# dantodor/Neural-Ficititious-Self-Play-in-Imperfect-Information-Games

Hardware: NVIDIA B200
Metric: leduc_transitions_per_sec (higher is better)
Workload: dtype f32

## Files before the change

include/nfsp_b200.h:

```cpp
#ifndef NFSP_B200_H
#define NFSP_B200_H
#include <stdint.h>

#ifdef __cplusplus
extern "C" {
#endif

#define NFSP_OK 0
#define NFSP_E_ARG (-1)
#define NFSP_E_CUDA (-2)
#define NFSP_E_STATE (-3)

#define NFSP_RULES_LEGACY 0
#define NFSP_RULES_NFSP 1

#define NFSP_OBS_DIM 30
#define NFSP_ACTIONS 3
#define NFSP_HIDDEN 64
#define NFSP_NET_PARAMS 2179
#define NFSP_EXPORT_FIELDS 24
#define NFSP_LEGACY_EXPORT_FIELDS 14
#define NFSP_STATS_FIELDS 16

typedef struct nfsp_env_s *nfsp_env_t;

int nfsp_version(void);
const char *nfsp_last_error(void);
int nfsp_device_info(int device, int *sm_count, int *cc_major, int *cc_minor, char *name, int name_len);

int nfsp_env_create(int rules, int64_t n_games, uint64_t seed, uint64_t game0, int device, nfsp_env_t *out);
int nfsp_env_destroy(nfsp_env_t h);
int64_t nfsp_env_num_games(nfsp_env_t h);
int nfsp_env_rules(nfsp_env_t h);
uint64_t nfsp_env_step_counter(nfsp_env_t h);
int nfsp_env_set_step_counter(nfsp_env_t h, uint64_t step);
void *nfsp_env_state_ptr(nfsp_env_t h);
int nfsp_env_kernel_error(nfsp_env_t h, uint32_t *out);
int nfsp_env_save_state(nfsp_env_t h, uint64_t *d_out, void *stream);
int nfsp_env_load_state(nfsp_env_t h, const uint64_t *d_in, void *stream);

int nfsp_env_reset(nfsp_env_t h, const int8_t *d_dealer, double eta, void *stream);
int nfsp_env_set_hands(nfsp_env_t h, const int8_t *d_dealer, const int8_t *d_cards, const int8_t *d_policy,
                       void *stream);
int nfsp_env_step(nfsp_env_t h, const int8_t *d_actions, const int8_t *d_players, int n_steps, int auto_reset,
                  double eta, uint32_t *d_trace, void *stream);
int nfsp_fsm_image(uint32_t *out, int capacity_words);
int nfsp_legacy_fsm_image(uint32_t *out, int capacity_words, int *n_rows);
int nfsp_rollout_image(uint32_t *out, int capacity_words);
int nfsp_env_do_action(nfsp_env_t h, const int8_t *d_actions, const int8_t *d_players, int8_t *d_fold, void *stream);
int nfsp_env_observe(nfsp_env_t h, const int8_t *d_players, int player, uint32_t *d_s, uint32_t *d_s2,
                     float *d_reward, uint8_t *d_term, uint8_t *d_last_a, void *stream);
int nfsp_env_export(nfsp_env_t h, int32_t *d_fields, void *stream);

int nfsp_legacy_reset(nfsp_env_t h, void *stream);
int nfsp_legacy_set_hands(nfsp_env_t h, const int8_t *d_cards, void *stream);
int nfsp_legacy_step(nfsp_env_t h, const int8_t *d_actions, const int8_t *d_players, int player, void *stream);
int nfsp_legacy_get_new_state(nfsp_env_t h, const int8_t *d_players, int player, int32_t *d_out, void *stream);
int nfsp_legacy_rollout(nfsp_env_t h, const int8_t *d_actions, int n_iters, uint32_t *d_rec, void *stream);
int nfsp_legacy_export(nfsp_env_t h, int32_t *d_fields, void *stream);

int nfsp_expand_obs(const uint32_t *d_masks, int64_t n, float *d_out, void *stream);

int nfsp_act_set_weights(nfsp_env_t h, const float *d_weights, void *stream);
int nfsp_act_set_weights_from_host(nfsp_env_t h, const float *h_weights, float *d_weights, void *stream);
int nfsp_act_forward(nfsp_env_t h, const uint32_t *d_obs, const int8_t *d_net, int64_t n, float *d_out,
                     void *stream);

int nfsp_act_forward_tc(nfsp_env_t h, const uint32_t *d_obs, const int8_t *d_net, int64_t n, float *d_out,
                        void *stream);

typedef struct {
    void *d_rl[2];
    void *d_sl[2];
    int64_t cap_rl, cap_sl;
    int32_t n_segments;
    uint32_t *d_counts;
    uint64_t *d_stats;
    uint32_t *d_trace;
    float *d_vec;
    const float *d_forced_vec;
    int32_t variant;
    int32_t reserve_sms;
    void *d_ring[2];
    uint64_t *d_ring_total[2];
    int64_t ring_cap;
    int32_t epsilon_per_player;
    double epsilon_p1;
} nfsp_rollout_io;
#define NFSP_ROLLOUT_DEFAULT_VARIANT 6

int nfsp_rollout(nfsp_env_t h, int n_steps, double eta, double epsilon, const nfsp_rollout_io *io, void *stream);
int nfsp_rollout_with_weights(nfsp_env_t h, const float *h_weights, float *d_weights, int n_steps, double eta, double epsilon,
                              const nfsp_rollout_io *io, void *stream);
int nfsp_rollout_tune(nfsp_env_t h, int patience_avg, int patience_br);
int nfsp_rollout_profile(nfsp_env_t h, uint64_t *out24);

#define NFSP_INSERT_SCRATCH_WORDS 4
int nfsp_ring_insert(void *d_ring, int64_t cap, uint64_t *d_total, const void *d_recs, uint32_t *d_counts,
                     int n_segments, int64_t seg_cap, uint64_t *d_scratch, void *stream);
#define NFSP_RESERVOIR_SLOT_BYTES 32
int nfsp_reservoir_insert(void *d_res, int64_t cap, uint64_t *d_total, const void *d_recs, uint32_t *d_counts,
                          int n_segments, int64_t seg_cap, uint64_t seed, int mode, uint64_t *d_scratch, void *stream);
#define NFSP_MAX_INSERT_REQS 4
typedef struct {
    void *d_mem;
    int64_t cap;
    uint64_t *d_total;
    uint64_t *d_scratch;
    const void *d_recs;
    uint32_t *d_counts;
    int32_t n_segments;
    int64_t seg_cap;
    uint64_t seed;
    int32_t mode;
    int32_t reservoir;
} nfsp_insert_req;
int nfsp_insert_multi(const nfsp_insert_req *reqs, int n, void *stream);
int nfsp_ring_insert_multi(const nfsp_insert_req *reqs, int n, void *stream);
int nfsp_reservoir_insert_multi(const nfsp_insert_req *reqs, int n, void *stream);
int nfsp_sample_indices(uint64_t seed, uint64_t call_idx, const uint64_t *d_total, int64_t cap, int is_ring,
                        int batch, int64_t *d_idx, uint32_t *d_n_out, void *stream);
#define NFSP_MAX_SAMPLE_REQS 8
typedef struct {
    const void *d_mem;
    const uint64_t *d_total;
    int64_t cap;
    uint64_t seed, call_idx;
    int32_t is_ring;
    float *d_out;
    void *d_rec_out;
} nfsp_sample_req;
int nfsp_sample_minibatches(const nfsp_sample_req *reqs, int n_reqs, int batch, int64_t *d_idx, uint32_t *d_n_out,
                            void *stream);
int nfsp_gather_rl(const void *d_ring, const int64_t *d_idx, int batch, float *d_s, float *d_a, float *d_r,
                   float *d_s2, float *d_t, void *stream);
int nfsp_gather_sl(const void *d_res, const int64_t *d_idx, int batch, float *d_s, float *d_a, void *stream);

#define NFSP_LEARNER_STATS 8
typedef struct {
    const float *d_weights;
    const float *d_target_weights;
    const void *d_rl[2];
    const int64_t *d_rl_idx[2];
    const void *d_sl[2];
    const int64_t *d_sl_idx[2];
    int32_t row0, rows;
    float gamma;
    int32_t net_mask;
    int32_t terminal_bootstraps;
    int32_t others_to_target;
    float *d_grad;
    float *d_stats;
} nfsp_learner_io;
int nfsp_learner_grads(const nfsp_learner_io *io, void *stream);
#define NFSP_MAX_FIT_STEPS 64
int nfsp_learner_fit(const nfsp_learner_io *io, int minibatch, int fit_batch, int epochs, const float lr[4],
                     float *d_weights_out, void *stream);
#define NFSP_MAX_PEERS 8
#define NFSP_PEER_BUF_FLOATS 279552
typedef struct {
    int32_t world, rank;
    void *d_buf[NFSP_MAX_PEERS];
    uint32_t epoch0;
    uint32_t *d_err;
    void *d_mc;
} nfsp_peers;
int nfsp_learner_fit_peers(const nfsp_learner_io *io, int minibatch, int fit_batch, int epochs, const float lr[4],
                           float *d_weights_out, const nfsp_peers *peers, void *stream);
int nfsp_peer_buffer_create(int device, void **d_buf, unsigned char *handle64);
int nfsp_peer_buffer_open(int device, const unsigned char *handle64, void **d_buf);
int nfsp_peer_buffer_close(int device, void *d_buf);
int nfsp_peer_buffer_destroy(int device, void *d_buf);
int nfsp_sgd_apply(float *d_weights, const float *d_grad, const float lr[4], float scale, void *stream);

#ifdef __cplusplus
}
#endif
#endif
```

neural-ficititious-self-play-in-imperfect-information-games_b200/_lib.py:

```python
from __future__ import annotations

import ctypes as C
import os

PKG_DIR = os.path.dirname(os.path.abspath(__file__))
LIB_PATH = os.path.join(PKG_DIR, "libnfsp_b200.so")

RULES_LEGACY, RULES_NFSP = 0, 1
OBS_DIM, ACTIONS, HIDDEN, NET_PARAMS = 30, 3, 64, 2179
EXPORT_FIELDS, LEGACY_EXPORT_FIELDS, STATS_FIELDS = 24, 14, 16

SYMBOLS = [
    "nfsp_version", "nfsp_last_error", "nfsp_device_info",
    "nfsp_env_create", "nfsp_env_destroy", "nfsp_env_num_games", "nfsp_env_rules", "nfsp_env_step_counter",
    "nfsp_env_set_step_counter", "nfsp_env_state_ptr", "nfsp_env_kernel_error", "nfsp_env_save_state", "nfsp_env_load_state",
    "nfsp_env_reset", "nfsp_env_set_hands", "nfsp_env_step", "nfsp_env_do_action", "nfsp_fsm_image", "nfsp_legacy_fsm_image", "nfsp_rollout_image", "nfsp_env_observe", "nfsp_env_export",
    "nfsp_legacy_reset", "nfsp_legacy_set_hands", "nfsp_legacy_step", "nfsp_legacy_get_new_state",
    "nfsp_legacy_rollout", "nfsp_legacy_export",
    "nfsp_expand_obs",
    "nfsp_act_set_weights", "nfsp_act_set_weights_from_host", "nfsp_act_forward", "nfsp_act_forward_tc", "nfsp_rollout", "nfsp_rollout_with_weights", "nfsp_rollout_tune", "nfsp_rollout_profile",
    "nfsp_ring_insert", "nfsp_reservoir_insert", "nfsp_insert_multi", "nfsp_ring_insert_multi", "nfsp_reservoir_insert_multi", "nfsp_sample_indices", "nfsp_sample_minibatches", "nfsp_gather_rl", "nfsp_gather_sl",
    "nfsp_learner_grads", "nfsp_learner_fit", "nfsp_learner_fit_peers", "nfsp_sgd_apply",
    "nfsp_peer_buffer_create", "nfsp_peer_buffer_open", "nfsp_peer_buffer_close", "nfsp_peer_buffer_destroy",
]


class RolloutIO(C.Structure):
    _fields_ = [("d_rl", C.c_void_p * 2), ("d_sl", C.c_void_p * 2), ("cap_rl", C.c_int64), ("cap_sl", C.c_int64),
                ("n_segments", C.c_int32), ("d_counts", C.c_void_p), ("d_stats", C.c_void_p), ("d_trace", C.c_void_p), ("d_vec", C.c_void_p),
                ("d_forced_vec", C.c_void_p), ("variant", C.c_int32), ("reserve_sms", C.c_int32),
                ("d_ring", C.c_void_p * 2), ("d_ring_total", C.c_void_p * 2), ("ring_cap", C.c_int64),
                ("epsilon_per_player", C.c_int32), ("epsilon_p1", C.c_double)]


class InsertReq(C.Structure):
    _fields_ = [("d_mem", C.c_void_p), ("cap", C.c_int64), ("d_total", C.c_void_p), ("d_scratch", C.c_void_p),
                ("d_recs", C.c_void_p), ("d_counts", C.c_void_p), ("n_segments", C.c_int32), ("seg_cap", C.c_int64),
                ("seed", C.c_uint64), ("mode", C.c_int32), ("reservoir", C.c_int32)]


INSERT_SCRATCH_WORDS, RESERVOIR_SLOT_BYTES = 4, 32


MAX_PEERS, PEER_BUF_FLOATS = 8, 279552


class Peers(C.Structure):
    _fields_ = [("world", C.c_int32), ("rank", C.c_int32), ("d_buf", C.c_void_p * MAX_PEERS), ("epoch0", C.c_uint32),
                ("d_err", C.c_void_p), ("d_mc", C.c_void_p)]


class SampleReq(C.Structure):
    _fields_ = [("d_mem", C.c_void_p), ("d_total", C.c_void_p), ("cap", C.c_int64), ("seed", C.c_uint64),
                ("call_idx", C.c_uint64), ("is_ring", C.c_int32), ("d_out", C.c_void_p), ("d_rec_out", C.c_void_p)]


class LearnerIO(C.Structure):
    _fields_ = [("d_weights", C.c_void_p), ("d_target_weights", C.c_void_p), ("d_rl", C.c_void_p * 2),
                ("d_rl_idx", C.c_void_p * 2), ("d_sl", C.c_void_p * 2), ("d_sl_idx", C.c_void_p * 2),
                ("row0", C.c_int32), ("rows", C.c_int32), ("gamma", C.c_float), ("net_mask", C.c_int32),
                ("terminal_bootstraps", C.c_int32), ("others_to_target", C.c_int32), ("d_grad", C.c_void_p), ("d_stats", C.c_void_p)]


class NfspError(RuntimeError):
    pass


_lib = None


def lib():
    global _lib
    if _lib is not None:
        return _lib
    if not os.path.exists(LIB_PATH):
        raise NfspError("libnfsp_b200.so is not built (%s): run `python -c 'import __graft_entry__ as g; g.build()'`; "
                        "there is no CPU fallback" % LIB_PATH)
    L = C.CDLL(LIB_PATH)
    vp, i8p = C.c_void_p, C.c_void_p
    L.nfsp_version.restype = C.c_int
    L.nfsp_last_error.restype = C.c_char_p
    L.nfsp_device_info.argtypes = [C.c_int, C.POINTER(C.c_int), C.POINTER(C.c_int), C.POINTER(C.c_int), C.c_char_p,
                                   C.c_int]
    L.nfsp_env_create.argtypes = [C.c_int, C.c_int64, C.c_uint64, C.c_uint64, C.c_int, C.POINTER(vp)]
    L.nfsp_env_destroy.argtypes = [vp]
    L.nfsp_env_num_games.argtypes = [vp]
    L.nfsp_env_num_games.restype = C.c_int64
    L.nfsp_env_rules.argtypes = [vp]
    L.nfsp_env_step_counter.argtypes = [vp]
    L.nfsp_env_step_counter.restype = C.c_uint64
    L.nfsp_env_set_step_counter.argtypes = [vp, C.c_uint64]
    L.nfsp_env_state_ptr.argtypes = [vp]
    L.nfsp_env_state_ptr.restype = vp
    L.nfsp_env_kernel_error.argtypes = [vp, C.POINTER(C.c_uint32)]
    L.nfsp_rollout_tune.argtypes = [vp, C.c_int, C.c_int]
    L.nfsp_rollout_profile.argtypes = [vp, C.POINTER(C.c_uint64)]
    L.nfsp_env_save_state.argtypes = [vp, vp, vp]
    L.nfsp_env_load_state.argtypes = [vp, vp, vp]
    L.nfsp_env_reset.argtypes = [vp, i8p, C.c_double, vp]
    L.nfsp_env_set_hands.argtypes = [vp, i8p, i8p, i8p, vp]
    L.nfsp_env_step.argtypes = [vp, i8p, i8p, C.c_int, C.c_int, C.c_double, vp, vp]
    L.nfsp_env_do_action.argtypes = [vp, i8p, i8p, i8p, vp]
    L.nfsp_fsm_image.argtypes = [vp, C.c_int]
    L.nfsp_legacy_fsm_image.argtypes = [vp, C.c_int, vp]
    L.nfsp_rollout_image.argtypes = [vp, C.c_int]
    L.nfsp_env_observe.argtypes = [vp, i8p, C.c_int, vp, vp, vp, vp, vp, vp]
    L.nfsp_env_export.argtypes = [vp, vp, vp]
    L.nfsp_legacy_reset.argtypes = [vp, vp]
    L.nfsp_legacy_set_hands.argtypes = [vp, i8p, vp]
    L.nfsp_legacy_step.argtypes = [vp, i8p, i8p, C.c_int, vp]
    L.nfsp_legacy_get_new_state.argtypes = [vp, i8p, C.c_int, vp, vp]
    L.nfsp_legacy_rollout.argtypes = [vp, i8p, C.c_int, vp, vp]
    L.nfsp_legacy_export.argtypes = [vp, vp, vp]
    L.nfsp_expand_obs.argtypes = [vp, C.c_int64, vp, vp]
    L.nfsp_act_set_weights.argtypes = [vp, vp, vp]
    L.nfsp_act_set_weights_from_host.argtypes = [vp, vp, vp, vp]
    L.nfsp_act_forward.argtypes = [vp, vp, i8p, C.c_int64, vp, vp]
    L.nfsp_act_forward_tc.argtypes = [vp, vp, i8p, C.c_int64, vp, vp]
    L.nfsp_rollout.argtypes = [vp, C.c_int, C.c_double, C.c_double, C.POINTER(RolloutIO), vp]
    L.nfsp_rollout_with_weights.argtypes = [vp, vp, vp, C.c_int, C.c_double, C.c_double, C.POINTER(RolloutIO), vp]
    L.nfsp_ring_insert.argtypes = [vp, C.c_int64, vp, vp, vp, C.c_int, C.c_int64, vp, vp]
    L.nfsp_reservoir_insert.argtypes = [vp, C.c_int64, vp, vp, vp, C.c_int, C.c_int64, C.c_uint64, C.c_int, vp, vp]
    L.nfsp_insert_multi.argtypes = [C.POINTER(InsertReq), C.c_int, vp]
    L.nfsp_ring_insert_multi.argtypes = [C.POINTER(InsertReq), C.c_int, vp]
    L.nfsp_reservoir_insert_multi.argtypes = [C.POINTER(InsertReq), C.c_int, vp]
    L.nfsp_sample_indices.argtypes = [C.c_uint64, C.c_uint64, vp, C.c_int64, C.c_int, C.c_int, vp, vp, vp]
    L.nfsp_sample_minibatches.argtypes = [C.POINTER(SampleReq), C.c_int, C.c_int, vp, vp, vp]
    L.nfsp_gather_rl.argtypes = [vp, vp, C.c_int, vp, vp, vp, vp, vp, vp]
    L.nfsp_gather_sl.argtypes = [vp, vp, C.c_int, vp, vp, vp]
    L.nfsp_learner_grads.argtypes = [C.POINTER(LearnerIO), vp]
    L.nfsp_learner_fit.argtypes = [C.POINTER(LearnerIO), C.c_int, C.c_int, C.c_int, C.POINTER(C.c_float), vp, vp]
    L.nfsp_learner_fit_peers.argtypes = [C.POINTER(LearnerIO), C.c_int, C.c_int, C.c_int, C.POINTER(C.c_float), vp,
                                         C.POINTER(Peers), vp]
    L.nfsp_sgd_apply.argtypes = [vp, vp, C.POINTER(C.c_float * 4), C.c_float, vp]
    L.nfsp_peer_buffer_create.argtypes = [C.c_int, C.POINTER(vp), C.c_char_p]
    L.nfsp_peer_buffer_open.argtypes = [C.c_int, C.c_char_p, C.POINTER(vp)]
    L.nfsp_peer_buffer_close.argtypes = [C.c_int, vp]
    L.nfsp_peer_buffer_destroy.argtypes = [C.c_int, vp]
    _lib = L
    return L


def check(rc: int):
    if rc != 0:
        raise NfspError("libnfsp_b200 error %d: %s" % (rc, lib().nfsp_last_error().decode("utf-8", "replace")))
```

neural-ficititious-self-play-in-imperfect-information-games_b200/csrc/act_kernels.cu:

```cuda
#include "mlp_math.cuh"
#include "ptx_helpers.cuh"
#include "rollout_fast.cuh"
#include "rollout_tables.cuh"

namespace nfsp {

constexpr int kActThreads = 128;
constexpr int kRollThreads = 1024;
constexpr int kFwdRowQuads = 24;
constexpr int kW1Floats = 128 * kFwdRowQuads * 4;
constexpr int kW2Floats = 4 * 3 * kFwdRowQuads * 4;
constexpr int kPackFloats = kW1Floats + kW2Floats + kB2Floats;

__device__ __forceinline__ float pack_weights_value(const float *__restrict__ w, int e) {
    {
        float v = 0.f;
        if (e < kW1Floats) {
            const int c = e & 3, pos = (e >> 2) % kFwdRowQuads, row = (e >> 2) / kFwdRowQuads;
            const int net = row >> 5, i = row & 31, j = (pos & 15) * 4 + c;
            const float *wn = w + net * NFSP_NET_PARAMS;
            if (i < 30) v = wn[i * 64 + j];
            else if (i == 30) v = wn[1920 + j];
        } else if (e < kW1Floats + kW2Floats) {
            const int f = e - kW1Floats, x = f & 3, pos = (f >> 2) % kFwdRowQuads, c = ((f >> 2) / kFwdRowQuads) % 3;
            const int net = (f >> 2) / (3 * kFwdRowQuads);
            v = w[net * NFSP_NET_PARAMS + 1984 + ((pos & 15) * 4 + x) * 3 + c];
        } else {
            const int f = e - kW1Floats - kW2Floats, c = f & 3, net = f >> 2;
            if (c < 3) v = w[net * NFSP_NET_PARAMS + 2176 + c];
        }
        return v;
    }
}

static_assert((kPackFloats + kTabImageFloats + 4 * NFSP_NET_PARAMS) % 4 == 0, "the state table behind the images must be 16-byte aligned (bulk copy)");
__global__ void pack_images_kernel(const float *__restrict__ w, float *__restrict__ pack) {
    constexpr int kImages = kPackFloats + kTabImageFloats;
    for (int e = blockIdx.x * blockDim.x + threadIdx.x; e < kImages + 4 * NFSP_NET_PARAMS; e += gridDim.x * blockDim.x)
        pack[e] = e < kPackFloats ? pack_weights_value(w, e) : (e < kImages ? pack_tables_value(w, e - kPackFloats) : w[e - kImages]);
}

__device__ __forceinline__ void mlp_forward(const float *__restrict__ sw, uint32_t obs, int net, uint32_t rot, float out[3]) {
    const float4 *w1 = reinterpret_cast<const float4 *>(sw) + rot;
    float4 h[16];
#pragma unroll
    for (int q = 0; q < 16; ++q) h[q] = make_float4(0.f, 0.f, 0.f, 0.f);
    uint32_t bits = (obs & 0x3FFFFFFFu) | (1u << 30);
    while (bits) {
        const int i = __ffs(bits) - 1;
        bits &= bits - 1u;
        const float4 *r = w1 + (net * 32 + i) * kFwdRowQuads;
#pragma unroll
        for (int q = 0; q < 16; ++q) {
            const float4 v = r[q];
            h[q].x += v.x; h[q].y += v.y; h[q].z += v.z; h[q].w += v.w;
        }
    }
    const float4 *w2 = reinterpret_cast<const float4 *>(sw + kW1Floats) + net * (3 * kFwdRowQuads) + rot;
    Layer2Acc acc;
#pragma unroll
    for (int q = 0; q < 16; ++q)
        acc.quad(h[q].x, h[q].y, h[q].z, h[q].w, w2[q], w2[kFwdRowQuads + q], w2[2 * kFwdRowQuads + q]);
    acc.head(reinterpret_cast<const float4 *>(sw + kW1Floats + kW2Floats)[net], net & 1, out[0], out[1], out[2]);
}

__device__ __forceinline__ void load_pack(float *sw, const float *__restrict__ pack) {
    const float4 *src = reinterpret_cast<const float4 *>(pack);
    float4 *dst = reinterpret_cast<float4 *>(sw);
    for (int e = threadIdx.x; e < kPackFloats / 4; e += blockDim.x) dst[e] = src[e];
    __syncthreads();
}

__global__ void __launch_bounds__(kActThreads)
act_forward_kernel(const float *__restrict__ pack, const uint32_t *__restrict__ obs, const int8_t *__restrict__ net,
                   int64_t n, float *__restrict__ out) {
    extern __shared__ __align__(16) float sw[];
    load_pack(sw, pack);
    for (int64_t i = blockIdx.x * (int64_t)blockDim.x + threadIdx.x; i < n; i += (int64_t)gridDim.x * blockDim.x) {
        float v[3];
        mlp_forward(sw, obs[i], (int)(net[i] & 3), (uint32_t)i & 7u, v);
        out[3 * i] = v[0]; out[3 * i + 1] = v[1]; out[3 * i + 2] = v[2];
    }
}

template <bool kDebug, bool kDirect>
__global__ void __launch_bounds__(kRollThreads, 1)
rollout_kernel(const RolloutArgs A) {
    extern __shared__ __align__(128) float sw[];
    __shared__ unsigned long long s_stats[NFSP_STATS_FIELDS];
    __shared__ __align__(8) uint64_t s_bar;
    __shared__ FastLuts s_lut;
    __shared__ uint32_t s_next;
    if (threadIdx.x < NFSP_STATS_FIELDS) s_stats[threadIdx.x] = 0ull;
    s_lut.fill();
    const uint32_t bar = smem_u32(&s_bar);
    if (threadIdx.x == 0) {
        s_next = 0u;
        mbar_init(bar, 1);
        fence_mbar_init();
    }
    __syncthreads();
    if (threadIdx.x == 0) {
        mbar_expect_tx(bar, kTabImageBytes);
        constexpr uint32_t kChunk = 32768;
        for (uint32_t off = 0; off < (uint32_t)kTabImageBytes; off += kChunk) {
            const uint32_t len = (uint32_t)kTabImageBytes - off < kChunk ? (uint32_t)kTabImageBytes - off : kChunk;
            bulk_g2s(smem_u32(sw) + off, reinterpret_cast<const uint8_t *>(A.pack) + off, len, bar);
        }
    }
    bool image_ready = false;

    FastCounters c;
    const int64_t plane = (int64_t)A.n_steps * A.n;
    const uint32_t lane = threadIdx.x & 31u;
    const int64_t n_blocks = (A.n + 31) >> 5;
    for (;;) {
        uint32_t blk = 0;
        if (lane == 0) blk = blockIdx.x + gridDim.x * atomicAdd(&s_next, 1u);
        blk = __shfl_sync(0xFFFFFFFFu, blk, 0);
        if ((int64_t)blk >= n_blocks) break;
        const int64_t base = (int64_t)blk << 5;
        const int64_t i = base + lane;
        const bool live = i < A.n;
        const uint64_t game = A.game0 + (uint64_t)i;
        const uint32_t rot = (uint32_t)game & 7u;
        WarpStage W;
        W.init(A, (uint32_t)(base >> 5) & (A.n_seg - 1u), kDirect);
        NfspFast g;
        g.unpack(live ? A.state[i] : 0ull);
        for (int t = 0; t < A.n_steps; ++t) {
            FastDecision d;
            fast_begin(g, s_lut, A, game, A.step0 + (uint64_t)t, live, d, c);
            const uint32_t sg = g.sigma(), dl = g.dealer(), ca = (g.PA >> 11) & 3u;
            const uint32_t xrow = sg >= 9u ? 3u + ((((ca * 3u + g.pub()) * 2u + dl) << 2) | g.fin0()) : ca;
            const uint32_t yrow = 75u + dl * 18u + sg;
            float v0, v1, v2;
            if (!image_ready) {
                mbar_wait(bar, 0);
                image_ready = true;
            }
            mlp_forward_tables(sw, xrow, yrow, g.p() * 2u + (uint32_t)d.pol, rot, v0, v1, v2);
            if (d.random) { v0 = d.r0; v1 = d.r1; v2 = d.r2; }
            fast_finish<kDebug, kDirect>(g, s_lut, A, W, d, v0, v1, v2, live, (int64_t)t * A.n + i, plane, c);
            if ((t & 15) == 15) c.spill();
        }
        c.spill();
        if (live) A.state[i] = g.pack();
        c.wide.trans += live ? A.n_steps : 0;
    }
    if (!image_ready) mbar_wait(bar, 0);
    c.spill();
    if (A.stats) c.wide.commit(s_stats, A.stats);
}

}

using namespace nfsp;

extern "C" int nfsp_act_set_weights(nfsp_env_t h, const float *d_weights, void *stream) {
    NFSP_CHECK_ARG(h != nullptr && d_weights != nullptr, "null argument");
    NFSP_CHECK_ARG(h->rules == NFSP_RULES_NFSP, "acting nets need NFSP rules");
    DeviceGuard guard(h->device);
    if (!guard.ok) return set_error(NFSP_E_CUDA, "cannot select device %d", h->device);
    if (!h->d_wpack) {
        NFSP_CUDA(cudaMalloc(&h->d_wpack, sizeof(float) * (kPackFloats + kTabImageFloats + 4 * NFSP_NET_PARAMS + nfsp_states_floats())));
        h->d_wcopy = h->d_wpack + kPackFloats + kTabImageFloats;
        h->d_states = h->d_wpack + kPackFloats + kTabImageFloats + 4 * NFSP_NET_PARAMS;
        NFSP_CUDA(cudaMalloc(&h->d_work, sizeof(uint32_t)));
        NFSP_CUDA(cudaFuncSetAttribute(act_forward_kernel, cudaFuncAttributeMaxDynamicSharedMemorySize, (int)(kPackFloats * sizeof(float))));
        NFSP_CUDA(cudaFuncSetAttribute(rollout_kernel<true, false>, cudaFuncAttributeMaxDynamicSharedMemorySize, kTabImageBytes));
        NFSP_CUDA(cudaFuncSetAttribute(rollout_kernel<false, false>, cudaFuncAttributeMaxDynamicSharedMemorySize, kTabImageBytes));
        NFSP_CUDA(cudaFuncSetAttribute(rollout_kernel<true, true>, cudaFuncAttributeMaxDynamicSharedMemorySize, kTabImageBytes));
        NFSP_CUDA(cudaFuncSetAttribute(rollout_kernel<false, true>, cudaFuncAttributeMaxDynamicSharedMemorySize, kTabImageBytes));
        int rc = nfsp_rollout_sorted_configure();
        if (rc != NFSP_OK) return rc;
        rc = nfsp_rollout_pairs_configure();
        if (rc != NFSP_OK) return rc;
        rc = nfsp_rollout_states_configure();
        if (rc != NFSP_OK) return rc;
        rc = nfsp_states_upload_image(h->d_states);
        if (rc != NFSP_OK) return rc;
    }
    pack_images_kernel<<<(kPackFloats + kTabImageFloats + 4 * NFSP_NET_PARAMS + 255) / 256, 256, 0, (cudaStream_t)stream>>>(d_weights, h->d_wpack);
    NFSP_LAUNCH_CHECK();
    h->tc_dirty = h->tq_dirty = h->st_dirty = true;
    h->has_weights = true;
    return nfsp_states_ensure(h, h->d_wpack + kPackFloats, h->d_states, (cudaStream_t)stream);
}

int nfsp_ensure_tc_images(nfsp_env_t h, bool tq, cudaStream_t st) {
    if (h->tc_dirty) {
        const int rc = nfsp_pack_tc_image(h, h->d_wcopy, st);
        if (rc != NFSP_OK) return rc;
        h->tc_dirty = false;
    }
    if (tq && h->tq_dirty) {
        const int rc = nfsp_tq_set_weights(h, h->d_wcopy, st);
        if (rc != NFSP_OK) return rc;
        h->tq_dirty = false;
    }
    return NFSP_OK;
}

extern "C" int nfsp_act_set_weights_from_host(nfsp_env_t h, const float *h_weights, float *d_weights, void *stream) {
    NFSP_CHECK_ARG(h != nullptr && h_weights != nullptr && d_weights != nullptr, "null argument");
    DeviceGuard guard(h->device);
    if (!guard.ok) return set_error(NFSP_E_CUDA, "cannot select device %d", h->device);
    NFSP_CUDA(cudaMemcpyAsync(d_weights, h_weights, sizeof(float) * 4 * NFSP_NET_PARAMS, cudaMemcpyHostToDevice,
                              (cudaStream_t)stream));
    return nfsp_act_set_weights(h, d_weights, stream);
}

extern "C" int nfsp_act_forward(nfsp_env_t h, const uint32_t *d_obs, const int8_t *d_net, int64_t n, float *d_out,
                                void *stream) {
    NFSP_CHECK_ARG(h != nullptr && d_obs && d_net && d_out && n >= 0, "bad arguments");
    if (!h->has_weights) return set_error(NFSP_E_STATE, "nfsp_act_set_weights has not been called");
    if (n == 0) return NFSP_OK;
    DeviceGuard guard(h->device);
    if (!guard.ok) return set_error(NFSP_E_CUDA, "cannot select device %d", h->device);
    const int grid = grid_for(n, kActThreads, h->sm_count, 4);
    act_forward_kernel<<<grid, kActThreads, kPackFloats * sizeof(float), (cudaStream_t)stream>>>(h->d_wpack, d_obs, d_net, n, d_out);
    NFSP_LAUNCH_CHECK();
    return NFSP_OK;
}

int nfsp_rollout_direct_args(const nfsp_rollout_io *io, RolloutArgs &A, bool *direct) {
    for (int q = 0; q < 2; ++q) { A.ring[q] = nullptr; A.ring_total[q] = nullptr; }
    A.ring_cap = 0u;
    A.ring_magic = 0ull;
    *direct = io->d_ring[0] != nullptr || io->d_ring[1] != nullptr;
    if (!*direct) return NFSP_OK;
    NFSP_CHECK_ARG(io->d_ring[0] && io->d_ring[1] && io->d_ring_total[0] && io->d_ring_total[1],
                   "the direct ring append needs both rings and their totals");
    NFSP_CHECK_ARG(io->ring_cap > 1 && io->ring_cap < ((int64_t)1 << 32), "ring capacity out of range");
    NFSP_CHECK_ARG(2 * A.n * (int64_t)A.n_steps <= io->ring_cap,
                   "direct ring append needs 2 * n * n_steps <= ring capacity (a launch must not lap the ring)");
    for (int q = 0; q < 2; ++q) {
        A.ring[q] = (uint4 *)io->d_ring[q];
        A.ring_total[q] = (unsigned long long *)io->d_ring_total[q];
    }
    A.ring_cap = (uint32_t)io->ring_cap;
    A.ring_magic = ~0ull / (uint64_t)io->ring_cap;
    return NFSP_OK;
}

extern "C" int nfsp_rollout(nfsp_env_t h, int n_steps, double eta, double epsilon, const nfsp_rollout_io *io,
                            void *stream) {
    NFSP_CHECK_ARG(h != nullptr && io != nullptr, "null argument");
    NFSP_CHECK_ARG(h->rules == NFSP_RULES_NFSP, "rollout needs NFSP rules");
    NFSP_CHECK_ARG(n_steps >= 1 && n_steps <= 4096, "n_steps must be in [1,4096]");
    NFSP_CHECK_ARG(io->d_rl[0] && io->d_rl[1] && io->d_sl[0] && io->d_sl[1] && io->d_counts, "missing staging arrays");
    NFSP_CHECK_ARG(io->cap_rl > 0 && io->cap_sl > 0 && io->cap_rl < ((int64_t)1 << 32) && io->cap_sl < ((int64_t)1 << 32),
                   "staging capacity out of range");
    NFSP_CHECK_ARG(io->n_segments >= 1 && io->n_segments <= 65536 && (io->n_segments & (io->n_segments - 1)) == 0,
                   "n_segments must be a power of two in [1,65536]");
    if (!h->has_weights) return set_error(NFSP_E_STATE, "nfsp_act_set_weights has not been called");
    DeviceGuard guard(h->device);
    if (!guard.ok) return set_error(NFSP_E_CUDA, "cannot select device %d", h->device);
    RolloutArgs A;
    A.keys = philox_keys(h->seed);
    A.state = h->d_state; A.n = h->n; A.seed = h->seed; A.game0 = h->game0; A.step0 = h->step; A.n_steps = n_steps;
    A.eta_u32 = frac_u32(eta); A.eps_u32 = frac_u32(epsilon);
    A.eps1_u32 = io->epsilon_per_player ? frac_u32(io->epsilon_p1) : A.eps_u32;
    A.pack = h->d_wpack + kPackFloats;
    for (int q = 0; q < 2; ++q) { A.rl[q] = (uint4 *)io->d_rl[q]; A.sl[q] = (uint4 *)io->d_sl[q]; }
    A.cap_rl = io->cap_rl; A.cap_sl = io->cap_sl; A.n_seg = (uint32_t)io->n_segments; A.counts = io->d_counts;
    A.work = h->d_work;
    A.stats = (unsigned long long *)io->d_stats; A.trace = io->d_trace; A.vec = io->d_vec; A.forced = io->d_forced_vec;
    const bool debug = io->d_trace || io->d_vec || io->d_forced_vec;
    NFSP_CHECK_ARG(io->variant >= 0 && io->variant <= 6,
                   "variant must be 0 (default), 1 (CUDA cores), 2 (tcgen05, one tile per group), 3 (tcgen05, warp-specialised), "
                   "4 (CUDA cores, net-sorted groups), 5 (CUDA cores, two games per lane) or 6 (table of the nets' outputs per decision state)");
    const int variant = io->variant == 0 ? NFSP_ROLLOUT_DEFAULT_VARIANT : io->variant;
    NFSP_CHECK_ARG(io->reserve_sms >= 0 && io->reserve_sms < h->sm_count, "reserve_sms must be in [0, %d)", h->sm_count);
    bool direct = false;
    {
        const int rc = nfsp_rollout_direct_args(io, A, &direct);
        if (rc != NFSP_OK) return rc;
    }
    NFSP_CHECK_ARG(!direct || variant == 1 || variant >= 4, "the direct ring append (d_ring) exists in variants 1, 4, 5 and 6 only");
    if (variant == 6) {
        int rc = nfsp_states_ensure(h, h->d_wpack + kPackFloats, h->d_states, (cudaStream_t)stream);
        if (rc != NFSP_OK) return rc;
        A.pack = h->d_states;
        rc = nfsp_rollout_states_launch(h, A, io, debug, (cudaStream_t)stream);
        if (rc != NFSP_OK) return rc;
        h->step += (uint64_t)n_steps;
        return NFSP_OK;
    }
    if (variant == 5) {
        const int rc = nfsp_rollout_pairs_launch(h, A, io, debug, (cudaStream_t)stream);
        if (rc != NFSP_OK) return rc;
        h->step += (uint64_t)n_steps;
        return NFSP_OK;
    }
    if (variant == 4) {
        const int rc = nfsp_rollout_sorted_launch(h, A, io, debug, (cudaStream_t)stream);
        if (rc != NFSP_OK) return rc;
        h->step += (uint64_t)n_steps;
        return NFSP_OK;
    }
    if (variant == 2 || variant == 3) {
        const int rc = nfsp_ensure_tc_images(h, variant == 3, (cudaStream_t)stream);
        if (rc != NFSP_OK) return rc;
    }
    if (variant == 3) {
        const int rc = nfsp_rollout_tq_launch(h, A, debug, io->reserve_sms, (cudaStream_t)stream);
        if (rc != NFSP_OK) return rc;
        h->step += (uint64_t)n_steps;
        return NFSP_OK;
    }
    if (variant == 2) {
        const int rc = nfsp_rollout_tc_launch(h, A, debug, (cudaStream_t)stream);
        if (rc != NFSP_OK) return rc;
        h->step += (uint64_t)n_steps;
        return NFSP_OK;
    }
    const int grid = grid_for(h->n, 32, h->sm_count - io->reserve_sms, 1);
    if (debug && direct) rollout_kernel<true, true><<<grid, kRollThreads, kTabImageBytes, (cudaStream_t)stream>>>(A);
    else if (debug) rollout_kernel<true, false><<<grid, kRollThreads, kTabImageBytes, (cudaStream_t)stream>>>(A);
    else if (direct) rollout_kernel<false, true><<<grid, kRollThreads, kTabImageBytes, (cudaStream_t)stream>>>(A);
    else rollout_kernel<false, false><<<grid, kRollThreads, kTabImageBytes, (cudaStream_t)stream>>>(A);
    NFSP_LAUNCH_CHECK();
    h->step += (uint64_t)n_steps;
    return NFSP_OK;
}

extern "C" int nfsp_rollout_with_weights(nfsp_env_t h, const float *h_weights, float *d_weights, int n_steps, double eta,
                                         double epsilon, const nfsp_rollout_io *io, void *stream) {
    const int rc = h_weights ? nfsp_act_set_weights_from_host(h, h_weights, d_weights, stream) : nfsp_act_set_weights(h, d_weights, stream);
    if (rc != NFSP_OK) return rc;
    return nfsp_rollout(h, n_steps, eta, epsilon, io, stream);
}
```

neural-ficititious-self-play-in-imperfect-information-games_b200/csrc/buffer_kernels.cu:

```cuda
#include <cstdlib>

#include "common.cuh"
#include "philox.cuh"

namespace nfsp {

constexpr int kBufThreads = 256;

__device__ __forceinline__ uint64_t mulhi64(uint64_t a, uint64_t b) { return __umul64hi(a, b); }

struct Batch {
    const uint4 *recs;
    uint32_t *counts;
    uint32_t n_seg;
    uint64_t seg_cap;
};

struct Mem {
    uint4 *data;
    uint64_t cap;
    uint64_t *total;
    uint64_t *scratch;
    Batch B;
    uint64_t seed;
    int mode;
    int reservoir;
};
struct MemSet {
    Mem m[NFSP_MAX_INSERT_REQS];
    int n;
    uint32_t gx;
    uint64_t chunk;
    int small;
};
constexpr int kScratchHead = 2;
constexpr uint64_t kResChunk = 1ull << 21;

__device__ __forceinline__ void grid_sync(uint64_t *ctrl) {
    __syncthreads();
    if (threadIdx.x == 0) {
        unsigned long long *cnt = reinterpret_cast<unsigned long long *>(ctrl);
        volatile unsigned long long *gen = reinterpret_cast<volatile unsigned long long *>(ctrl + 1);
        const unsigned long long g = *gen;
        __threadfence();
        if (atomicAdd(cnt, 1ull) == (unsigned long long)gridDim.x - 1ull) {
            *cnt = 0ull;
            __threadfence();
            atomicAdd(const_cast<unsigned long long *>(gen), 1ull);
        } else {
            while (*gen == g) __nanosleep(32);
        }
        __threadfence();
    }
    __syncthreads();
}

__device__ __forceinline__ void scan_counts(const Mem &M) {
    __shared__ unsigned long long s_warp[kBufThreads / 32];
    __shared__ unsigned long long s_run;
    if (threadIdx.x == 0) s_run = 0ull;
    __syncthreads();
    uint64_t *pre = M.scratch + kScratchHead;
    const uint32_t lane = threadIdx.x & 31u, warp = threadIdx.x >> 5;
    for (uint32_t k0 = 0; k0 < M.B.n_seg; k0 += kBufThreads) {
        const uint32_t k = k0 + threadIdx.x;
        unsigned long long c = 0ull;
        if (k < M.B.n_seg) {
            c = M.B.counts[k];
            if (c > M.B.seg_cap) c = M.B.seg_cap;
        }
        unsigned long long incl = c;
#pragma unroll
        for (int o = 1; o < 32; o <<= 1) {
            const unsigned long long up = __shfl_up_sync(0xFFFFFFFFu, incl, o);
            if (lane >= (uint32_t)o) incl += up;
        }
        if (lane == 31) s_warp[warp] = incl;
        __syncthreads();
        unsigned long long before = s_run;
        for (uint32_t w = 0; w < warp; ++w) before += s_warp[w];
        if (k < M.B.n_seg) pre[k] = before + incl - c;
        __syncthreads();
        if (threadIdx.x == kBufThreads - 1) s_run = before + incl;
        __syncthreads();
    }
    if (threadIdx.x == 0) pre[M.B.n_seg] = s_run;
}

constexpr int kRingUnroll = 4;
__device__ __forceinline__ void ring_item(const Mem &M, uint64_t total, uint32_t seg, uint32_t x, uint32_t gx, uint64_t before,
                                          uint64_t cnt, uint64_t m) {
    const Batch &B = M.B;
    const uint64_t cap = M.cap;
    const uint64_t first = m > cap ? m - cap : 0;
    const uint4 *src = B.recs + (uint64_t)seg * B.seg_cap;
    uint4 *ring = M.data;
    const uint64_t head = total % cap;
    const uint64_t stride = (uint64_t)gx * blockDim.x;
    for (uint64_t i0 = x * (uint64_t)blockDim.x + threadIdx.x; i0 < cnt; i0 += stride * kRingUnroll) {
        uint4 v[kRingUnroll];
#pragma unroll
        for (int u = 0; u < kRingUnroll; ++u) {
            const uint64_t i = i0 + (uint64_t)u * stride;
            if (i < cnt) v[u] = __ldcs(src + i);
        }
#pragma unroll
        for (int u = 0; u < kRingUnroll; ++u) {
            const uint64_t i = i0 + (uint64_t)u * stride, idx = before + i;
            if (i < cnt && idx >= first) {
                uint64_t slot = head + idx;
                if (slot >= cap) slot -= cap;
                if (slot >= cap) slot %= cap;
                ring[slot] = v[u];
            }
        }
    }
}

__device__ __forceinline__ int64_t reservoir_slot(uint64_t seed, uint64_t ticket, uint64_t cap, int mode) {
    if (ticket < cap) return (int64_t)ticket;
    const uint64_t u = buffer_u64(seed, ticket, 0, STREAM_RESERVOIR);
    if (mode == 1) {
        const uint64_t j = 1u + mulhi64(u, cap);
        return j < cap ? (int64_t)j : -1;
    }
    const uint64_t j = mulhi64(u, ticket + 1u);
    return j < cap ? (int64_t)j : -1;
}

constexpr int kResUnroll = 4;

template <bool kWrite>
__device__ __forceinline__ void reservoir_item(const Mem &M, uint64_t total, uint32_t seg, uint32_t x, uint32_t gx, uint64_t lo,
                                               uint64_t hi, uint64_t before, uint64_t cnt) {
    const Batch &B = M.B;
    if (before >= hi || before + cnt <= lo) return;
    const uint64_t i_lo = lo > before ? lo - before : 0, i_hi = hi - before < cnt ? hi - before : cnt;
    const uint64_t cap = M.cap, seed = M.seed;
    const int mode = M.mode;
    uint4 *res = M.data;
    const uint4 *src = B.recs + (uint64_t)seg * B.seg_cap;
    const uint64_t stride = (uint64_t)gx * blockDim.x;
    for (uint64_t i0 = i_lo + x * (uint64_t)blockDim.x + threadIdx.x; i0 < i_hi; i0 += stride * kResUnroll) {
        int64_t slot[kResUnroll];
#pragma unroll
        for (int u = 0; u < kResUnroll; ++u) {
            const uint64_t i = i0 + (uint64_t)u * stride;
            slot[u] = i < i_hi ? reservoir_slot(seed, total + before + i, cap, mode) : -1;
        }
        if (!kWrite) {
#pragma unroll
            for (int u = 0; u < kResUnroll; ++u)
                if (slot[u] >= 0)
                    atomicMax(reinterpret_cast<unsigned long long *>(res + 2 * slot[u] + 1),
                              (unsigned long long)(total + before + i0 + (uint64_t)u * stride + 1u));
        } else {
            unsigned long long owner[kResUnroll];
#pragma unroll
            for (int u = 0; u < kResUnroll; ++u)
                owner[u] = slot[u] >= 0 ? __ldcg(reinterpret_cast<const unsigned long long *>(res + 2 * slot[u] + 1)) : 0ull;
#pragma unroll
            for (int u = 0; u < kResUnroll; ++u) {
                const uint64_t i = i0 + (uint64_t)u * stride;
                if (slot[u] >= 0 && owner[u] == (unsigned long long)(total + before + i + 1u)) res[2 * slot[u]] = __ldcs(src + i);
            }
        }
    }
}

template <class F>
__device__ __forceinline__ void for_items(const MemSet &S, int k, const uint64_t *pre, bool in_smem, F f) {
    const uint64_t items = (uint64_t)S.m[k].B.n_seg * S.gx;
    for (uint64_t w = blockIdx.x; w < items; w += gridDim.x) {
        const uint32_t seg = (uint32_t)(w / S.gx), x = (uint32_t)(w % S.gx);
        const uint64_t before = in_smem ? pre[seg] : __ldcg(pre + seg), next = in_smem ? pre[seg + 1] : __ldcg(pre + seg + 1);
        f(seg, x, before, next - before);
    }
}

constexpr int kSmallSegs = 32;

__global__ void __launch_bounds__(kBufThreads, 4) insert_kernel(const MemSet S) {
    __shared__ uint64_t s_pre[NFSP_MAX_INSERT_REQS][kSmallSegs + 1];
    uint64_t *ctrl = S.m[0].scratch;
    uint64_t total[NFSP_MAX_INSERT_REQS], m_all[NFSP_MAX_INSERT_REQS];
    const uint64_t *pre[NFSP_MAX_INSERT_REQS];
    const bool small = S.small != 0;
#pragma unroll
    for (int k = 0; k < NFSP_MAX_INSERT_REQS; ++k) total[k] = k < S.n ? *S.m[k].total : 0ull;
    if (small) {
        const uint32_t lane = threadIdx.x & 31u, warp = threadIdx.x >> 5;
        if (warp < (uint32_t)S.n) {
            const Mem &M = S.m[warp];
            unsigned long long c = lane < M.B.n_seg ? (unsigned long long)__ldcg(M.B.counts + lane) : 0ull;
            if (c > M.B.seg_cap) c = M.B.seg_cap;
            unsigned long long incl = c;
#pragma unroll
            for (int o = 1; o < 32; o <<= 1) {
                const unsigned long long up = __shfl_up_sync(0xFFFFFFFFu, incl, o);
                if (lane >= (uint32_t)o) incl += up;
            }
            s_pre[warp][lane + 1] = incl;
            if (lane == 0) s_pre[warp][0] = 0ull;
        }
        __syncthreads();
#pragma unroll
        for (int k = 0; k < NFSP_MAX_INSERT_REQS; ++k) {
            pre[k] = s_pre[k];
            m_all[k] = k < S.n ? s_pre[k][S.m[k].B.n_seg] : 0ull;
        }
    } else {
        for (int k = blockIdx.x; k < S.n; k += gridDim.x) scan_counts(S.m[k]);
        grid_sync(ctrl);
#pragma unroll
        for (int k = 0; k < NFSP_MAX_INSERT_REQS; ++k) {
            pre[k] = k < S.n ? S.m[k].scratch + kScratchHead : nullptr;
            m_all[k] = k < S.n ? __ldcg(pre[k] + S.m[k].B.n_seg) : 0ull;
        }
    }
    uint64_t res_max = 0;
#pragma unroll
    for (int k = 0; k < NFSP_MAX_INSERT_REQS; ++k)
        if (k < S.n && S.m[k].reservoir) res_max = m_all[k] > res_max ? m_all[k] : res_max;
#pragma unroll
    for (int k = 0; k < NFSP_MAX_INSERT_REQS; ++k)
        if (k < S.n && !S.m[k].reservoir)
            for_items(S, k, pre[k], small, [&](uint32_t seg, uint32_t x, uint64_t before, uint64_t cnt) {
                ring_item(S.m[k], total[k], seg, x, S.gx, before, cnt, m_all[k]);
            });
    for (uint64_t lo = 0; lo < res_max; lo += S.chunk) {
#pragma unroll
        for (int k = 0; k < NFSP_MAX_INSERT_REQS; ++k)
            if (k < S.n && S.m[k].reservoir)
                for_items(S, k, pre[k], small, [&](uint32_t seg, uint32_t x, uint64_t before, uint64_t cnt) {
                    reservoir_item<false>(S.m[k], total[k], seg, x, S.gx, lo, lo + S.chunk, before, cnt);
                });
        grid_sync(ctrl);
#pragma unroll
        for (int k = 0; k < NFSP_MAX_INSERT_REQS; ++k)
            if (k < S.n && S.m[k].reservoir)
                for_items(S, k, pre[k], small, [&](uint32_t seg, uint32_t x, uint64_t before, uint64_t cnt) {
                    reservoir_item<true>(S.m[k], total[k], seg, x, S.gx, lo, lo + S.chunk, before, cnt);
                });
    }
    if (small && res_max == 0) grid_sync(ctrl);
#pragma unroll
    for (int k = 0; k < NFSP_MAX_INSERT_REQS; ++k)
        if (k < S.n && (uint32_t)k % gridDim.x == blockIdx.x) {
            const Mem &M = S.m[k];
            for (uint32_t s = threadIdx.x; s < M.B.n_seg; s += blockDim.x) M.B.counts[s] = 0u;
            if (threadIdx.x == 0) *M.total = total[k] + m_all[k];
        }
}

constexpr int kMaxBatch = 1024;

template <class SlotT>
__device__ __forceinline__ int floyd_sample(uint64_t seed, uint64_t call_idx, uint64_t total, uint64_t cap, int is_ring,
                                            int batch, uint64_t *draw, uint64_t *pick, SlotT *slot_out) {
    __shared__ int s_collision;
    const uint64_t count = total < cap ? total : cap;
    const int b = (uint64_t)batch < count ? batch : (int)count;
    const uint64_t lo = count - (uint64_t)b;
    if (threadIdx.x == 0) s_collision = 0;
    for (int m = threadIdx.x; m < b; m += blockDim.x)
        draw[m] = mulhi64(buffer_u64(seed, (uint64_t)m, call_idx, STREAM_SAMPLE), lo + (uint64_t)m + 1u);
    __syncthreads();
    __shared__ unsigned char s_dup[kMaxBatch];
    for (int m = threadIdx.x; m < b; m += blockDim.x) {
        const uint64_t t = draw[m];
        bool dup = false;
        for (int k = 0; k < m; ++k) dup |= (draw[k] == t);
        if (dup) s_collision = 1;
        s_dup[m] = dup;
    }
    __syncthreads();
    while (s_collision) {
        __syncthreads();
        if (threadIdx.x == 0) s_collision = 0;
        __syncthreads();
        for (int m = threadIdx.x; m < b; m += blockDim.x) {
            const uint64_t t = draw[m];
            if (!s_dup[m] && t >= lo && t - lo < (uint64_t)m && s_dup[t - lo]) {
                s_dup[m] = 1;
                s_collision = 1;
            }
        }
        __syncthreads();
    }
    for (int m = threadIdx.x; m < b; m += blockDim.x) pick[m] = s_dup[m] ? lo + (uint64_t)m : draw[m];
    __syncthreads();
    const uint64_t head = (is_ring && total >= cap) ? total % cap : 0;
    for (int m = threadIdx.x; m < batch; m += blockDim.x) {
        int64_t slot = -1;
        if (m < b) slot = is_ring ? (int64_t)((head + pick[m]) % cap) : (int64_t)pick[m];
        slot_out[m] = (SlotT)slot;
    }
    return b;
}

__global__ void __launch_bounds__(kBufThreads)
sample_kernel(uint64_t seed, uint64_t call_idx, const uint64_t *__restrict__ total_p, uint64_t cap, int is_ring,
              int batch, int64_t *__restrict__ idx_out, uint32_t *__restrict__ n_out) {
    __shared__ uint64_t draw[kMaxBatch];
    __shared__ uint64_t pick[kMaxBatch];
    const int b = floyd_sample(seed, call_idx, *total_p, cap, is_ring, batch, draw, pick, idx_out);
    if (threadIdx.x == 0 && n_out) *n_out = (uint32_t)b;
}

__device__ __forceinline__ void expand_rl(const uint4 rec, int row, int col, float *__restrict__ s, float *__restrict__ a,
                                          float *__restrict__ r, float *__restrict__ s2, float *__restrict__ t) {
    if (col < 30) s[row * 30 + col] = (float)((rec.x >> col) & 1u);
    else if (col < 60) s2[row * 30 + (col - 30)] = (float)((rec.y >> (col - 30)) & 1u);
    else if (col < 63) a[row * 3 + (col - 60)] = ((rec.w & 0xFFu) == (uint32_t)(col - 60)) ? 1.f : 0.f;
    else if (col == 63) r[row] = __uint_as_float(rec.z);
    else t[row] = (float)((rec.w >> 8) & 0xFFu);
}
__device__ __forceinline__ void expand_sl(const uint4 rec, int row, int col, float *__restrict__ s, float *__restrict__ a) {
    if (col < 30) s[row * 30 + col] = (float)((rec.x >> col) & 1u);
    else a[row * 3 + (col - 30)] = __uint_as_float(col == 30 ? rec.y : (col == 31 ? rec.z : rec.w));
}

struct SampleReqs {
    const uint4 *mem[NFSP_MAX_SAMPLE_REQS];
    const uint64_t *total[NFSP_MAX_SAMPLE_REQS];
    uint64_t cap[NFSP_MAX_SAMPLE_REQS], seed[NFSP_MAX_SAMPLE_REQS], call_idx[NFSP_MAX_SAMPLE_REQS];
    float *out[NFSP_MAX_SAMPLE_REQS];
    uint4 *rec_out[NFSP_MAX_SAMPLE_REQS];
    int is_ring[NFSP_MAX_SAMPLE_REQS];
};
__global__ void __launch_bounds__(kBufThreads)
sample_gather_kernel(const SampleReqs R, int batch, int64_t *__restrict__ idx_out, uint32_t *__restrict__ n_out) {
    __shared__ uint64_t draw[kMaxBatch];
    __shared__ uint64_t pick[kMaxBatch];
    __shared__ int64_t slot[kMaxBatch];
    __shared__ uint4 s_rec[kMaxBatch];
    const int m = blockIdx.x;
    const int b = floyd_sample(R.seed[m], R.call_idx[m], *R.total[m], R.cap[m], R.is_ring[m], batch, draw, pick, slot);
    __syncthreads();
    const int per = (batch + (int)gridDim.y - 1) / (int)gridDim.y;
    const int row0 = (int)blockIdx.y * per, row1 = min(batch, row0 + per);
    if (threadIdx.x == 0 && blockIdx.y == 0 && n_out) n_out[m] = (uint32_t)b;
    const uint4 *mem = R.mem[m];
    float *o = R.out[m];
    uint4 *ro = R.rec_out[m];
    const int stride = R.is_ring[m] ? 1 : 2;
    for (int k = row0 + threadIdx.x; k < row1; k += blockDim.x) {
        if (idx_out) idx_out[(int64_t)m * batch + k] = slot[k];
        if (o || ro) {
            const uint4 rec = slot[k] >= 0 ? mem[slot[k] * stride] : make_uint4(0, 0, 0, 0);
            if (o) s_rec[k] = rec;
            if (ro) ro[k * stride] = rec;
        }
    }
    if (!o) return;
    __syncthreads();
    const int rows = max(row1 - row0, 0);
    if (R.is_ring[m]) {
        float *s = o, *a = s + 30 * batch, *r = a + 3 * batch, *s2 = r + batch, *t = s2 + 30 * batch;
        for (int e = threadIdx.x; e < rows * 65; e += blockDim.x) {
            const int row = row0 + e / 65, col = e % 65;
            expand_rl(s_rec[row], row, col, s, a, r, s2, t);
        }
    } else {
        float *s = o, *a = s + 30 * batch;
        for (int e = threadIdx.x; e < rows * 33; e += blockDim.x) {
            const int row = row0 + e / 33, col = e % 33;
            expand_sl(s_rec[row], row, col, s, a);
        }
    }
}

__global__ void __launch_bounds__(kBufThreads)
gather_rl_kernel(const uint4 *__restrict__ ring, const int64_t *__restrict__ idx, int batch, float *__restrict__ s,
                 float *__restrict__ a, float *__restrict__ r, float *__restrict__ s2, float *__restrict__ t) {
    const int total = batch * 65;
    for (int e = blockIdx.x * blockDim.x + threadIdx.x; e < total; e += gridDim.x * blockDim.x) {
        const int row = e / 65, col = e - row * 65;
        const int64_t slot = idx[row];
        expand_rl(slot >= 0 ? ring[slot] : make_uint4(0, 0, 0, 0), row, col, s, a, r, s2, t);
    }
}

__global__ void __launch_bounds__(kBufThreads)
gather_sl_kernel(const uint4 *__restrict__ res, const int64_t *__restrict__ idx, int batch, float *__restrict__ s,
                 float *__restrict__ a) {
    const int total = batch * 33;
    for (int e = blockIdx.x * blockDim.x + threadIdx.x; e < total; e += gridDim.x * blockDim.x) {
        const int row = e / 33, col = e - row * 33;
        const int64_t slot = idx[row];
        expand_sl(slot >= 0 ? res[2 * slot] : make_uint4(0, 0, 0, 0), row, col, s, a);
    }
}

}

using namespace nfsp;

static int make_memset(const nfsp_insert_req *reqs, int n, int want_kind, MemSet &S, int64_t *seg_cap_max) {
    NFSP_CHECK_ARG(reqs && n >= 1 && n <= NFSP_MAX_INSERT_REQS, "1..%d memories per call", NFSP_MAX_INSERT_REQS);
    *seg_cap_max = 0;
    int64_t rows = 0;
    for (int k = 0; k < NFSP_MAX_INSERT_REQS; ++k) S.m[k] = Mem{};
    for (int k = 0; k < n; ++k) {
        const nfsp_insert_req &r = reqs[k];
        NFSP_CHECK_ARG(r.d_mem && r.d_total && r.cap > 0, "bad memory %d", k);
        NFSP_CHECK_ARG(r.d_recs && r.d_counts && r.d_scratch, "null staged batch or scratch %d", k);
        NFSP_CHECK_ARG(r.n_segments >= 1 && r.n_segments <= 65535 && r.seg_cap >= 0, "bad segment geometry %d", k);
        NFSP_CHECK_ARG(r.reservoir == 0 || r.reservoir == 1, "reservoir must be 0 (ring) or 1 (reservoir)");
        NFSP_CHECK_ARG(want_kind < 0 || r.reservoir == want_kind, "memory %d is of the other kind", k);
        if (r.reservoir) NFSP_CHECK_ARG(r.mode == 0 || r.mode == 1, "mode must be 0 (Algorithm R) or 1 (reference law)");
        S.m[k].data = (uint4 *)r.d_mem;
        S.m[k].cap = (uint64_t)r.cap;
        S.m[k].total = r.d_total;
        S.m[k].scratch = r.d_scratch;
        S.m[k].B = Batch{(const uint4 *)r.d_recs, r.d_counts, (uint32_t)r.n_segments, (uint64_t)r.seg_cap};
        S.m[k].seed = r.seed;
        S.m[k].mode = r.mode;
        S.m[k].reservoir = r.reservoir;
        if (r.seg_cap > *seg_cap_max) *seg_cap_max = r.seg_cap;
        rows += r.n_segments;
    }
    S.n = n;
    int64_t g = (*seg_cap_max + kBufThreads - 1) / kBufThreads;
    const int64_t lim = rows >= 148 * 8 ? 1 : (148 * 8 + rows - 1) / rows;
    if (g > lim) g = lim;
    if (g < 1) g = 1;
    S.gx = (uint32_t)g;
    S.small = 1;
    for (int k = 0; k < n; ++k)
        if (reqs[k].n_segments > 32) S.small = 0;
    S.chunk = kResChunk;
#ifdef NFSP_TUNING_HOOKS
    if (const char *e = getenv("NFSP_RES_CHUNK")) {
        const long long v = atoll(e);
        if (v >= 1024) S.chunk = (uint64_t)v;
    }
#endif
    return NFSP_OK;
}

static int launch_insert(MemSet &S, cudaStream_t st) {
    int dev = 0, sms = 0, per_sm = 0;
    NFSP_CUDA(cudaGetDevice(&dev));
    NFSP_CUDA(cudaDeviceGetAttribute(&sms, cudaDevAttrMultiProcessorCount, dev));
    NFSP_CUDA(cudaOccupancyMaxActiveBlocksPerMultiprocessor(&per_sm, insert_kernel, kBufThreads, 0));
    if (per_sm < 1) return set_error(NFSP_E_CUDA, "insert_kernel does not fit an SM");
    if (per_sm > 8) per_sm = 8;
    int64_t items = 0;
    for (int k = 0; k < S.n; ++k) items += (int64_t)S.m[k].B.n_seg * S.gx;
    int64_t grid = (int64_t)sms * per_sm;
    if (items < grid) grid = items;
    if (grid < S.n) grid = S.n;
    void *args[] = {(void *)&S};
    NFSP_CUDA(cudaLaunchCooperativeKernel((const void *)insert_kernel, dim3((unsigned)grid), dim3(kBufThreads), args, 0, st));
    return NFSP_OK;
}

extern "C" int nfsp_insert_multi(const nfsp_insert_req *reqs, int n, void *stream) {
    MemSet S;
    int64_t seg_cap;
    const int rc = make_memset(reqs, n, -1, S, &seg_cap);
    if (rc != NFSP_OK) return rc;
    if (seg_cap == 0) return NFSP_OK;
    return launch_insert(S, (cudaStream_t)stream);
}

extern "C" int nfsp_ring_insert_multi(const nfsp_insert_req *reqs, int n, void *stream) {
    MemSet S;
    int64_t seg_cap;
    const int rc = make_memset(reqs, n, 0, S, &seg_cap);
    if (rc != NFSP_OK) return rc;
    if (seg_cap == 0) return NFSP_OK;
    return launch_insert(S, (cudaStream_t)stream);
}

extern "C" int nfsp_reservoir_insert_multi(const nfsp_insert_req *reqs, int n, void *stream) {
    MemSet S;
    int64_t seg_cap;
    const int rc = make_memset(reqs, n, 1, S, &seg_cap);
    if (rc != NFSP_OK) return rc;
    if (seg_cap == 0) return NFSP_OK;
    return launch_insert(S, (cudaStream_t)stream);
}

extern "C" int nfsp_ring_insert(void *d_ring, int64_t cap, uint64_t *d_total, const void *d_recs, uint32_t *d_counts,
                                int n_segments, int64_t seg_cap, uint64_t *d_scratch, void *stream) {
    nfsp_insert_req r{};
    r.d_mem = d_ring; r.cap = cap; r.d_total = d_total; r.d_recs = d_recs; r.d_counts = d_counts;
    r.n_segments = n_segments; r.seg_cap = seg_cap; r.d_scratch = d_scratch;
    return nfsp_ring_insert_multi(&r, 1, stream);
}

extern "C" int nfsp_reservoir_insert(void *d_res, int64_t cap, uint64_t *d_total, const void *d_recs, uint32_t *d_counts,
                                     int n_segments, int64_t seg_cap, uint64_t seed, int mode, uint64_t *d_scratch,
                                     void *stream) {
    nfsp_insert_req r{};
    r.d_mem = d_res; r.cap = cap; r.d_total = d_total; r.d_recs = d_recs; r.d_counts = d_counts;
    r.n_segments = n_segments; r.seg_cap = seg_cap; r.seed = seed; r.mode = mode; r.d_scratch = d_scratch; r.reservoir = 1;
    return nfsp_reservoir_insert_multi(&r, 1, stream);
}

extern "C" int nfsp_sample_indices(uint64_t seed, uint64_t call_idx, const uint64_t *d_total, int64_t cap,
                                   int is_ring, int batch, int64_t *d_idx, uint32_t *d_n_out, void *stream) {
    NFSP_CHECK_ARG(d_total && d_idx && cap > 0, "bad arguments");
    NFSP_CHECK_ARG(batch >= 1 && batch <= kMaxBatch, "batch must be in [1,%d]", kMaxBatch);
    sample_kernel<<<1, kBufThreads, 0, (cudaStream_t)stream>>>(seed, call_idx, d_total, (uint64_t)cap, is_ring, batch,
                                                               d_idx, d_n_out);
    NFSP_LAUNCH_CHECK();
    return NFSP_OK;
}

extern "C" int nfsp_sample_minibatches(const nfsp_sample_req *reqs, int n_reqs, int batch, int64_t *d_idx, uint32_t *d_n_out,
                                       void *stream) {
    NFSP_CHECK_ARG(reqs && n_reqs >= 1 && n_reqs <= NFSP_MAX_SAMPLE_REQS, "1..%d requests", NFSP_MAX_SAMPLE_REQS);
    NFSP_CHECK_ARG(batch >= 1 && batch <= kMaxBatch, "batch must be in [1,%d]", kMaxBatch);
    SampleReqs R;
    for (int m = 0; m < n_reqs; ++m) {
        NFSP_CHECK_ARG(reqs[m].d_mem && reqs[m].d_total && reqs[m].cap > 0, "bad request %d", m);
        NFSP_CHECK_ARG(reqs[m].d_out || reqs[m].d_rec_out || d_idx, "request %d has neither an output block nor an index array", m);
        R.mem[m] = (const uint4 *)reqs[m].d_mem;
        R.total[m] = reqs[m].d_total;
        R.cap[m] = (uint64_t)reqs[m].cap;
        R.seed[m] = reqs[m].seed;
        R.call_idx[m] = reqs[m].call_idx;
        R.out[m] = reqs[m].d_out;
        R.rec_out[m] = (uint4 *)reqs[m].d_rec_out;
        R.is_ring[m] = reqs[m].is_ring;
    }
    sample_gather_kernel<<<dim3((unsigned)n_reqs, 8u, 1u), kBufThreads, 0, (cudaStream_t)stream>>>(R, batch, d_idx, d_n_out);
    NFSP_LAUNCH_CHECK();
    return NFSP_OK;
}

extern "C" int nfsp_gather_rl(const void *d_ring, const int64_t *d_idx, int batch, float *d_s, float *d_a, float *d_r,
                              float *d_s2, float *d_t, void *stream) {
    NFSP_CHECK_ARG(d_ring && d_idx && d_s && d_a && d_r && d_s2 && d_t && batch >= 1, "bad arguments");
    gather_rl_kernel<<<(batch * 65 + kBufThreads - 1) / kBufThreads, kBufThreads, 0, (cudaStream_t)stream>>>(
        (const uint4 *)d_ring, d_idx, batch, d_s, d_a, d_r, d_s2, d_t);
    NFSP_LAUNCH_CHECK();
    return NFSP_OK;
}

extern "C" int nfsp_gather_sl(const void *d_res, const int64_t *d_idx, int batch, float *d_s, float *d_a,
                              void *stream) {
    NFSP_CHECK_ARG(d_res && d_idx && d_s && d_a && batch >= 1, "bad arguments");
    gather_sl_kernel<<<(batch * 33 + kBufThreads - 1) / kBufThreads, kBufThreads, 0, (cudaStream_t)stream>>>(
        (const uint4 *)d_res, d_idx, batch, d_s, d_a);
    NFSP_LAUNCH_CHECK();
    return NFSP_OK;
}
```

neural-ficititious-self-play-in-imperfect-information-games_b200/csrc/common.cuh:

```cuda
#pragma once
#include <cuda_runtime.h>

#include <cstdarg>
#include <cstdint>
#include <cstdio>

#include "../../include/nfsp_b200.h"

struct nfsp_env_s {
    int rules;
    int device;
    int sm_count;
    int64_t n;
    uint64_t seed, game0, step;
    uint64_t *d_state;
    uint32_t *d_fsm;
    float *d_wpack;
    uint32_t *d_work;
    void *d_wtc_wide;
    bool has_weights;
    bool tc_dirty = false, tq_dirty = false;
    bool st_dirty = false;
    float *d_states = nullptr;
    const float *d_wcopy = nullptr;
    int w2_slot = -1;
    void *d_w2img = nullptr;
    uint32_t *d_err = nullptr;
    uint32_t tq_patience[2] = {1500u, 700u};
};

int nfsp_fsm_upload(nfsp_env_t h);

int nfsp_pack_tc_image(nfsp_env_t h, const float *d_weights, cudaStream_t st);
int nfsp_ensure_tc_images(nfsp_env_t h, bool tq, cudaStream_t st);
int nfsp_tq_set_weights(nfsp_env_t h, const float *d_weights, cudaStream_t st);
void nfsp_tq_release(nfsp_env_t h);

namespace nfsp {

int set_error(int code, const char *fmt, ...);

#define NFSP_CHECK_ARG(cond, ...)                                    \
    do {                                                             \
        if (!(cond)) return nfsp::set_error(NFSP_E_ARG, __VA_ARGS__); \
    } while (0)

#define NFSP_CUDA(call)                                                                                   \
    do {                                                                                                  \
        cudaError_t e__ = (call);                                                                         \
        if (e__ != cudaSuccess)                                                                           \
            return nfsp::set_error(NFSP_E_CUDA, "%s failed: %s (%s:%d)", #call, cudaGetErrorString(e__), \
                                   __FILE__, __LINE__);                                                   \
    } while (0)

#define NFSP_LAUNCH_CHECK() NFSP_CUDA(cudaGetLastError())

inline uint32_t frac_u32(double x) {
    if (!(x > 0.0)) return 0u;
    const double v = x * 4294967296.0;
    return v >= 4294967295.0 ? 0xFFFFFFFFu : (uint32_t)v;
}

inline int grid_for(int64_t n, int threads, int sm_count, int ctas_per_sm) {
    const int64_t need = (n + threads - 1) / threads;
    const int64_t full = (int64_t)sm_count * ctas_per_sm;
    int64_t g = need < full ? need : full;
    if (g < 1) g = 1;
    return (int)g;
}

struct DeviceGuard {
    int prev = -1;
    bool ok = true;
    explicit DeviceGuard(int dev) {
        if (cudaGetDevice(&prev) != cudaSuccess) ok = false;
        if (ok && prev != dev && cudaSetDevice(dev) != cudaSuccess) ok = false;
    }
    ~DeviceGuard() {
        if (prev >= 0) cudaSetDevice(prev);
    }
};

}
```

neural-ficititious-self-play-in-imperfect-information-games_b200/csrc/ptx_helpers.cuh:

```cuda
#pragma once
#include <cstdint>

namespace nfsp {

__device__ __forceinline__ uint32_t smem_u32(const void *p) { return (uint32_t)__cvta_generic_to_shared(p); }

__device__ __forceinline__ void mbar_init(uint32_t bar, uint32_t count) {
    asm volatile("mbarrier.init.shared::cta.b64 [%0], %1;" ::"r"(bar), "r"(count));
}
__device__ __forceinline__ void mbar_expect_tx(uint32_t bar, uint32_t bytes) {
    asm volatile("mbarrier.arrive.expect_tx.shared::cta.b64 _, [%0], %1;" ::"r"(bar), "r"(bytes) : "memory");
}
__device__ __forceinline__ void mbar_wait(uint32_t bar, uint32_t parity) {
    asm volatile(
        "{\n\t"
        ".reg .pred p;\n\t"
        "WAIT_%=:\n\t"
        "mbarrier.try_wait.parity.shared::cta.b64 p, [%0], %1;\n\t"
        "@p bra DONE_%=;\n\t"
        "bra WAIT_%=;\n\t"
        "DONE_%=:\n\t"
        "}" ::"r"(bar), "r"(parity) : "memory");
}
__device__ __forceinline__ void mbar_wait_backoff(uint32_t bar, uint32_t parity) {
    uint32_t done = 0;
    while (true) {
        asm volatile(
            "{\n\t"
            ".reg .pred p;\n\t"
            "mbarrier.try_wait.parity.shared::cta.b64 p, [%1], %2;\n\t"
            "selp.u32 %0, 1, 0, p;\n\t"
            "}" : "=r"(done) : "r"(bar), "r"(parity) : "memory");
        if (done) break;
        __nanosleep(64);
    }
}
__device__ __forceinline__ void bulk_g2s(uint32_t dst, const void *src, uint32_t bytes, uint32_t bar) {
    asm volatile("cp.async.bulk.shared::cluster.global.mbarrier::complete_tx::bytes [%0], [%1], %2, [%3];" ::"r"(dst),
                 "l"(src), "r"(bytes), "r"(bar)
                 : "memory");
}
__device__ __forceinline__ void fence_mbar_init() { asm volatile("fence.mbarrier_init.release.cluster;" ::: "memory"); }

}
```

neural-ficititious-self-play-in-imperfect-information-games_b200/csrc/rollout_common.cuh:

```cuda
#pragma once
#include "common.cuh"
#include "nfsp_rules.cuh"
#include "philox.cuh"

namespace nfsp { struct RolloutArgs; }
int nfsp_rollout_tc_launch(nfsp_env_t h, const nfsp::RolloutArgs &A, bool debug, cudaStream_t st);
int nfsp_rollout_tq_launch(nfsp_env_t h, const nfsp::RolloutArgs &A, bool debug, int reserve_sms, cudaStream_t st);

int nfsp_rollout_sorted_launch(nfsp_env_t h, const nfsp::RolloutArgs &A, const nfsp_rollout_io *io, bool debug, cudaStream_t st);
int nfsp_rollout_direct_args(const nfsp_rollout_io *io, nfsp::RolloutArgs &A, bool *direct);
int nfsp_rollout_sorted_configure();
int nfsp_rollout_pairs_launch(nfsp_env_t h, const nfsp::RolloutArgs &A, const nfsp_rollout_io *io, bool debug, cudaStream_t st);
int nfsp_rollout_pairs_configure();

int nfsp_rollout_states_launch(nfsp_env_t h, const nfsp::RolloutArgs &A, const nfsp_rollout_io *io, bool debug, cudaStream_t st);
int nfsp_states_ensure(nfsp_env_t h, const float *d_tab, float *d_states, cudaStream_t st);
int nfsp_states_floats();
int nfsp_states_upload_image(float *d_states);
int nfsp_rollout_states_configure();

namespace nfsp {

struct RolloutArgs {
    uint64_t *state;
    int64_t n;
    uint64_t seed, game0, step0;
    PhiloxKeys keys;
    int n_steps;
    uint32_t eta_u32, eps_u32, eps1_u32;
    const void *pack;
    uint4 *rl[2];
    uint4 *sl[2];
    int64_t cap_rl, cap_sl;
    uint32_t n_seg;
    uint32_t *counts;
    uint32_t *work;
    unsigned long long *stats;
    uint32_t *trace;
    float *vec;
    const float *forced;
    uint4 *ring[2];
    unsigned long long *ring_total[2];
    uint32_t ring_cap;
    uint64_t ring_magic;
};

__device__ __forceinline__ uint32_t ring_slot(unsigned long long ticket, uint32_t cap, uint64_t magic) {
    const unsigned long long q = __umul64hi(ticket, magic);
    unsigned long long r = ticket - q * cap;
    if (r >= cap) r -= cap;
    return (uint32_t)r;
}

struct Counters {
    unsigned long long act0 = 0ull, act1 = 0ull;
    int rew0 = 0, rew1 = 0, hands = 0, trans = 0, drop = 0;

    __device__ __forceinline__ void commit(unsigned long long *s_stats, unsigned long long *g_stats) {
        long long v[11] = {(long long)(act0 & 0x1FFFFFull), (long long)((act0 >> 21) & 0x1FFFFFull), (long long)(act0 >> 42),
                           (long long)(act1 & 0x1FFFFFull), (long long)((act1 >> 21) & 0x1FFFFFull), (long long)(act1 >> 42),
                           rew0, rew1, hands, trans, drop};
#pragma unroll
        for (int k = 0; k < 11; ++k) {
#pragma unroll
            for (int o = 16; o > 0; o >>= 1) v[k] += __shfl_xor_sync(0xFFFFFFFFu, v[k], o);
        }
        if ((threadIdx.x & 31) == 0) {
#pragma unroll
            for (int k = 0; k < 11; ++k)
                if (v[k]) atomicAdd(&s_stats[k < 6 ? k : k + 2], (unsigned long long)v[k]);
        }
        act0 = act1 = 0ull;
        __syncthreads();
        if (threadIdx.x == 6) s_stats[6] = s_stats[0] + s_stats[1] + s_stats[2];
        if (threadIdx.x == 7) s_stats[7] = s_stats[3] + s_stats[4] + s_stats[5];
        __syncthreads();
        if (threadIdx.x < 13 && s_stats[threadIdx.x]) atomicAdd(g_stats + threadIdx.x, s_stats[threadIdx.x]);
    }
};

}
```

neural-ficititious-self-play-in-imperfect-information-games_b200/csrc/rollout_states.cu:

```cuda
#include "nfsp_fsm.cuh"
#include "rollout_fast.cuh"
#include "rollout_tables.cuh"
#include "ptx_helpers.cuh"

namespace nfsp {

constexpr int kNetStates = 72 * 18;
constexpr int kStateQuads = 4 * kNetStates;
constexpr int kStateBytes = kStateQuads * 16;
static_assert(kStateBytes % 16 == 0, "bulk copies move multiples of 16 bytes");
static_assert(kNetStates == fsm::kNetSlots, "the rollout image addresses this table");

__device__ __forceinline__ uint32_t score_word(float v0, float v1, float v2) {
    const uint32_t an = score_action(v0, v1, v2);
    return (an & 3u) * (uint32_t)fsm::kEntryBytes | (an >> 2) << 15;
}
constexpr uint32_t kWordEntry = 0x60u, kWordNz = 1u << 15;

__device__ __forceinline__ void state_rows(int s, uint32_t &xrow, uint32_t &yrow) {
    const uint32_t sg = (uint32_t)s % 18u, x = (uint32_t)s / 18u, dl = (x >> 2) & 1u;
    xrow = sg >= 9u ? 3u + x : x / 24u;
    yrow = 75u + dl * 18u + sg;
}

__global__ void states_pack_kernel(const float *__restrict__ tab, float4 *__restrict__ states) {
    const int t = blockIdx.x * blockDim.x + threadIdx.x, e = t >> 2, j = t & 3;
    const bool valid = e < kStateQuads;
    uint32_t xrow, yrow;
    state_rows(valid ? e % kNetStates : 0, xrow, yrow);
    const uint32_t net = valid ? (uint32_t)(e / kNetStates) : 0u;
    const float4 *T = reinterpret_cast<const float4 *>(tab);
    const float4 *xr = T + (net * kNetRows + xrow) * kRowQuads, *yr = T + (net * kNetRows + yrow) * kRowQuads;
    const float4 *wr = T + kTabRows * kRowQuads + net * (3 * kRowQuads);
    Layer2Acc acc;
#pragma unroll
    for (int k = 0; k < 4; ++k) {
        const int q = j + 4 * k;
        acc.quad_sum(xr[q], yr[q], wr[q], wr[kRowQuads + q], wr[2 * kRowQuads + q]);
    }
    float s0 = hsum2(acc.z0), s1 = hsum2(acc.z1), s2 = hsum2(acc.z2);
#pragma unroll
    for (int o = 1; o < 4; o <<= 1) {
        s0 += __shfl_xor_sync(0xFFFFFFFFu, s0, o);
        s1 += __shfl_xor_sync(0xFFFFFFFFu, s1, o);
        s2 += __shfl_xor_sync(0xFFFFFFFFu, s2, o);
    }
    if (valid && j == 0) {
        float o0, o1, o2;
        Layer2Acc::head_of_sums(s0, s1, s2, reinterpret_cast<const float4 *>(tab + kTabFloats + kTabW2Floats)[net], net & 1u, o0, o1, o2);
        states[e] = make_float4(o0, o1, o2, __uint_as_float(score_word(o0, o1, o2)));
    }
}

constexpr int kStatesThreads = 1024, kStatesThreadsSmall = 512;

constexpr int kBufRL = 100, kBufSL = 32;
constexpr int kWarpBufQuads = 2 * kBufRL + 2 * kBufSL;
constexpr int kImageQuads = fsm::kRImageBytes / 16;
constexpr int states_smem_bytes(int threads) { return kStateBytes + fsm::kRImageBytes + (threads / 32) * kWarpBufQuads * 16; }
static_assert(fsm::kRImageBytes % 16 == 0, "the warps' buffers follow the image 16-byte aligned");
static_assert(kBufRL >= 64 && kBufSL >= 32, "a buffer must take the records of one step");

constexpr uint32_t kOffRL1 = kBufRL, kOffSL0 = 2 * kBufRL, kOffSL1 = 2 * kBufRL + kBufSL;

struct WarpBuf {
    uint4 *b;
    uint32_t cnt = 0u;
};

__device__ __forceinline__ uint32_t warp_scan_bytes_p(uint32_t v) {
#pragma unroll
    for (int o = 1; o < 32; o <<= 1)
        asm volatile("{ .reg .pred p; .reg .u32 r; shfl.sync.up.b32 r|p, %0, %1, 0, 0xffffffff; @p add.u32 %0, %0, r; }" : "+r"(v) : "r"(o));
    return v;
}

template <bool kRing, int kCap>
__device__ __forceinline__ void buf_copy(const uint4 *src, uint32_t n, uint4 *dst, uint32_t base, uint32_t cap, int &drop) {
    const uint32_t lane = threadIdx.x & 31u;
#pragma unroll
    for (int it = 0; it < (kCap + 31) / 32; ++it) {
        const uint32_t k = lane + 32u * it;
        if (k < n) {
            uint32_t off = base + k;
            if (kRing) {
                off = off < cap ? off : off - cap;
                dst[off] = src[k];
            } else if (off < cap) {
                dst[off] = src[k];
            } else {
                ++drop;
            }
        }
    }
}

template <bool kDirect>
__device__ __forceinline__ void buf_flush(WarpBuf &B, const RolloutArgs &A, const WarpStage &W, FastCounters &c, uint32_t which) {
    __syncwarp();
    const uint32_t lane = threadIdx.x & 31u;
    uint32_t base = 0u;
    if (lane < 4u) {
        const uint32_t n = (B.cnt >> (8u * lane)) & 0xFFu;
        if (n && ((which >> lane) & 1u)) {
            if (kDirect && lane < 2u) base = ring_slot(atomicAdd(A.ring_total[lane], (unsigned long long)n), A.ring_cap, A.ring_magic);
            else base = atomicAdd(W.cnt + lane * W.n_seg, n);
        }
    }
    const uint32_t b0 = __shfl_sync(0xFFFFFFFFu, base, 0), b1 = __shfl_sync(0xFFFFFFFFu, base, 1);
    const uint32_t b2 = __shfl_sync(0xFFFFFFFFu, base, 2), b3 = __shfl_sync(0xFFFFFFFFu, base, 3);
    int drop = 0;
    if (which & 1u) buf_copy<kDirect, kBufRL>(B.b, B.cnt & 0xFFu, W.rl0, b0, W.cap_rl, drop);
    if (which & 2u) buf_copy<kDirect, kBufRL>(B.b + kOffRL1, (B.cnt >> 8) & 0xFFu, W.rl1, b1, W.cap_rl, drop);
    if (which & 4u) buf_copy<false, kBufSL>(B.b + kOffSL0, (B.cnt >> 16) & 0xFFu, W.sl0, b2, W.cap_sl, drop);
    if (which & 8u) buf_copy<false, kBufSL>(B.b + kOffSL1, B.cnt >> 24, W.sl1, b3, W.cap_sl, drop);
    c.wide.drop += drop;
    B.cnt &= ~(((which & 1u) ? 0xFFu : 0u) | ((which & 2u) ? 0xFF00u : 0u) | ((which & 4u) ? 0xFF0000u : 0u) | ((which & 8u) ? 0xFF000000u : 0u));
    __syncwarp();
}

template <bool kDirect>
__device__ __forceinline__ void buf_append(WarpBuf &B, const RolloutArgs &A, const WarpStage &W, FastCounters &c, uint32_t q,
                                           bool vA, bool vB, bool vC, bool vS, const uint4 &recA, const uint4 &recB,
                                           const uint4 &recC, const uint4 &recS) {
    const uint32_t rel = ((uint32_t)vA + (uint32_t)vB) | (uint32_t)vC << 8 | (uint32_t)vS << 16;
    const uint32_t mine = q ? __byte_perm(rel, 0u, 0x2301u) : rel;
    const uint32_t incl = warp_scan_bytes_p(mine);
    const uint32_t tot = __shfl_sync(0xFFFFFFFFu, incl, 31);
    constexpr uint32_t kOverRL = 127u - (uint32_t)kBufRL, kOverSL = 127u - (uint32_t)kBufSL;
    const uint32_t over = (B.cnt + tot + (kOverRL | kOverRL << 8 | kOverSL << 16 | kOverSL << 24)) & 0x80808080u;
    if (over) {
        uint32_t which = ((over >> 7) & 1u) | ((over >> 14) & 2u) | ((over >> 21) & 4u) | ((over >> 28) & 8u);
        if (which & 3u) which |= 3u;
        buf_flush<kDirect>(B, A, W, c, which);
    }
    const uint32_t pos = B.cnt + (incl - mine);
    const uint32_t prel = q ? __byte_perm(pos, 0u, 0x2301u) : pos;
    uint32_t own = q * kOffRL1 + (prel & 0xFFu);
    if (vA) B.b[own++] = recA;
    if (vB) B.b[own] = recB;
    if (vC) B.b[(q ^ 1u) * kOffRL1 + ((prel >> 8) & 0xFFu)] = recC;
    if (vS) B.b[kOffSL0 + q * (uint32_t)kBufSL + ((prel >> 16) & 0xFFu)] = recS;
    B.cnt += tot;
}

template <bool kDebug, bool kDirect, int kThreads>
__global__ void __launch_bounds__(kThreads, 1)
rollout_states_kernel(const RolloutArgs A) {
    extern __shared__ __align__(128) float4 s_tab[];
    __shared__ unsigned long long s_stats[NFSP_STATS_FIELDS];
    __shared__ __align__(8) uint64_t s_bar;
    __shared__ uint32_t s_next;
    if (threadIdx.x < NFSP_STATS_FIELDS) s_stats[threadIdx.x] = 0ull;
    const uint32_t sbase = smem_u32(s_tab), ibase = sbase + (uint32_t)kStateBytes;
    {
        const uint32_t *img = reinterpret_cast<const uint32_t *>(A.pack) + 4 * kStateQuads;
        uint32_t *dst = reinterpret_cast<uint32_t *>(s_tab + kStateQuads);
        for (int w = threadIdx.x; w < fsm::kRImageWords; w += kThreads) dst[w] = img[w] + (fsm::is_rollout_address(w) ? sbase : 0u);
    }
    const uint32_t bar = smem_u32(&s_bar);
    if (threadIdx.x == 0) {
        s_next = 0u;
        mbar_init(bar, 1);
        fence_mbar_init();
    }
    __syncthreads();
    if (threadIdx.x == 0) {
        mbar_expect_tx(bar, kStateBytes);
        constexpr uint32_t kChunk = 32768;
        for (uint32_t off = 0; off < (uint32_t)kStateBytes; off += kChunk) {
            const uint32_t len = (uint32_t)kStateBytes - off < kChunk ? (uint32_t)kStateBytes - off : kChunk;
            bulk_g2s(sbase + off, reinterpret_cast<const uint8_t *>(A.pack) + off, len, bar);
        }
    }
    bool image_ready = false;
    const uint32_t dl_sum = 2u * (ibase + (uint32_t)fsm::kRDealOff) + (uint32_t)fsm::kRDealHalf;
    const uint32_t rew_base = ibase + (uint32_t)fsm::kRRewardOff;

    FastCounters c;
    const int64_t plane = (int64_t)A.n_steps * A.n;
    const uint32_t lane = threadIdx.x & 31u;
    WarpBuf B;
    B.b = reinterpret_cast<uint4 *>(s_tab) + kStateQuads + kImageQuads + __shfl_sync(0xFFFFFFFFu, (threadIdx.x >> 5) * (uint32_t)kWarpBufQuads, 0);
    WarpStage W;
    W.init(A, 0u, kDirect);
    const int64_t n_blocks = (A.n + 31) >> 5;
    for (;;) {
        uint32_t blk = 0;
        if (lane == 0) blk = blockIdx.x + gridDim.x * atomicAdd(&s_next, 1u);
        blk = __shfl_sync(0xFFFFFFFFu, blk, 0);
        if ((int64_t)blk >= n_blocks) break;
        const int64_t base = (int64_t)blk << 5;
        const int64_t i = base + lane;
        const bool live = i < A.n;
        const uint64_t game = A.game0 + (uint64_t)i;
        W.init(A, (uint32_t)(base >> 5) & (A.n_seg - 1u), kDirect);
        fsm::RolloutGame g;
        g.unpack(live ? A.state[i] : 0ull, ibase, sbase);
        if (!image_ready) {
            mbar_wait(bar, 0);
            image_ready = true;
        }
        for (int t = 0; t < A.n_steps; ++t) {
            const uint64_t step = A.step0 + (uint64_t)t;
            const Philox4 x = game_block(A.keys, game, step, STREAM_STEP);
            uint32_t started = 0u;
            if (g.HX & fsm::kHxOver) {
                g.dl = dl_sum - g.dl;
                const uint4 D = fsm::lds128(g.dl + __umulhi(x.y, 120u) * 16u);
                uint32_t pa = g.dl + (uint32_t)fsm::kPolOff;
                if (x.z < A.eta_u32) pa += 16u;
                if (x.w < A.eta_u32) pa += 32u;
                const uint4 P = fsm::lds128(pa);
                g.PA = D.x | P.x;
                g.PO = D.y | P.y;
                g.FA = D.z + P.z;
                g.FO = D.w + P.w;
                g.SA = 0u;
                g.SO = 0u;
                g.tix = g.dl - (uint32_t)fsm::kRDealOff;
                g.HX = fsm::kCm0;
                started = 1u;
                c.wide.hands += live;
            }
            const uint32_t q = (g.PA >> 23) & 1u;
            const uint32_t obs = g.HX & (g.PA | 0x00FFFFFFu);
            const bool vA = (g.PA & kWordNz) != 0u, pol = (g.PA & (1u << 12)) != 0u;
            const uint4 recA = make_uint4(g.SA, obs, 0u, ((g.PA >> 13) & 3u) | (q << 16));
            const uint4 o = fsm::lds128(g.FA);
            float v0 = __uint_as_float(o.x), v1 = __uint_as_float(o.y), v2 = __uint_as_float(o.z);
            uint32_t aw = o.w;
            if (pol && x.x < (q ? A.eps1_u32 : A.eps_u32)) {
                const Philox4 y = game_block(A.keys, game, step, STREAM_VECTOR);
                v0 = (float)(y.x >> 8) * (1.0f / 16777216.0f);
                v1 = (float)(y.y >> 8) * (1.0f / 16777216.0f);
                v2 = (float)(y.z >> 8) * (1.0f / 16777216.0f);
                aw = score_word(v0, v1, v2);
            }
            const int64_t at = (int64_t)t * A.n + i;
            if (kDebug && live) {
                if (A.vec) { A.vec[3 * at] = v0; A.vec[3 * at + 1] = v1; A.vec[3 * at + 2] = v2; }
                if (A.forced) { v0 = A.forced[3 * at]; v1 = A.forced[3 * at + 1]; v2 = A.forced[3 * at + 2]; }
                aw = score_word(v0, v1, v2);
            }
            const uint32_t ea = g.tix + (aw & kWordEntry);
            const uint4 E = fsm::lds128(ea);
            const uint4 M = fsm::lds128(ea + 16u);
            g.PA = ((g.PA & ~fsm::kPClear) | (aw & kWordNz)) + E.y;
            g.HX = (g.HX & 0xFFFFFFu) | E.x;
            c.small += live ? M.w : 0u;
            const bool term = (g.HX & fsm::kHxOver) != 0u;
            const uint32_t rw = fsm::lds32(rew_base + (M.z & ((g.PA & 0xFFu) | (g.PO & 0xF00u))));
            const int ra = (int)(int8_t)(rw & 0xFFu), ro = (int)(int8_t)((rw >> 8) & 0xFFu);
            c.wide.rew0 += live ? (q ? ro : ra) : 0;
            c.wide.rew1 += live ? (q ? ra : ro) : 0;
            const float fa = 0.5f * (float)ra;
            const uint4 recB = make_uint4(obs, g.HX & (g.PA | 0x00FFFFFFu), __float_as_uint(fa), M.y & 0x10103u);
            const uint4 recC = make_uint4(g.SO, g.HX & (g.PO | 0x00FFFFFFu), __float_as_uint(0.5f * (float)ro),
                                          ((g.PO >> 13) & 3u) | ((M.y & 0x10100u) ^ 0x10000u));
            const bool vB = term && (aw & kWordNz) && live, vC = term && (g.PO & kWordNz) && live;
            if (kDebug && live && A.trace) {
                const uint32_t P0 = q ? g.PO : g.PA, P1 = q ? g.PA : g.PO;
                const uint32_t d = g.dl != ibase + (uint32_t)fsm::kRDealOff ? 1u : 0u;
                A.trace[at] = g.HX & (g.PA | 0xC0FFFFFFu);
                A.trace[plane + at] = __float_as_uint(fa);
                A.trace[2 * plane + at] = (M.y & 0x101Fu) | (d << 5) | (((P0 >> 19) & 3u) << 6) | (((P1 >> 19) & 3u) << 8) |
                                          (((P0 >> 21) & 3u) << 10) | (((P0 >> 2) & 15u) << 13) | (((P1 >> 2) & 15u) << 17) |
                                          (started << 21) | (((P0 >> 12) & 1u) << 22) | (((P1 >> 12) & 1u) << 23);
            }
            const uint32_t pm = E.z, pa = g.PA, sa = obs, fa_ = g.FA + M.x, fo = g.FO + M.x;
            g.PA = (g.PO & pm) | (pa & ~pm);
            g.PO = (pa & pm) | (g.PO & ~pm);
            g.SA = (g.SO & pm) | (sa & ~pm);
            g.SO = (sa & pm) | (g.SO & ~pm);
            g.FA = (fo & pm) | (fa_ & ~pm);
            g.FO = (fa_ & pm) | (fo & ~pm);
            g.tix = E.w;
            buf_append<kDirect>(B, A, W, c, q, vA && live, vB, vC, pol && live, recA, recB, recC,
                                make_uint4(obs, __float_as_uint(v0), __float_as_uint(v1), __float_as_uint(v2)));
            if ((t & 15) == 15) c.spill();
        }
        c.spill();
        if (live) A.state[i] = g.pack(ibase);
        c.wide.trans += live ? A.n_steps : 0;
        buf_flush<kDirect>(B, A, W, c, kDirect ? 12u : 15u);
    }
    if (kDirect) buf_flush<true>(B, A, W, c, 3u);
    if (!image_ready) mbar_wait(bar, 0);
    c.spill();
    if (A.stats) c.wide.commit(s_stats, A.stats);
}

}

using namespace nfsp;

int nfsp_states_floats() { return kStateQuads * 4 + fsm::kRImageWords; }

static void build_states_image(uint32_t *img) { fsm::build_rollout_image(img, (uint32_t)kStateBytes); }

int nfsp_states_upload_image(float *d_states) {
    static uint32_t image[fsm::kRImageWords];
    static const bool built = (build_states_image(image), true);
    (void)built;
    NFSP_CUDA(cudaMemcpy(d_states + 4 * kStateQuads, image, sizeof(image), cudaMemcpyHostToDevice));
    return NFSP_OK;
}

extern "C" int nfsp_rollout_image(uint32_t *out, int capacity_words) {
    if (out && capacity_words >= fsm::kRImageWords) build_states_image(out);
    return fsm::kRImageWords;
}

template <int kThreads>
static int configure_states() {
    constexpr int kBytes = states_smem_bytes(kThreads);
    NFSP_CUDA(cudaFuncSetAttribute(rollout_states_kernel<true, true, kThreads>, cudaFuncAttributeMaxDynamicSharedMemorySize, kBytes));
    NFSP_CUDA(cudaFuncSetAttribute(rollout_states_kernel<true, false, kThreads>, cudaFuncAttributeMaxDynamicSharedMemorySize, kBytes));
    NFSP_CUDA(cudaFuncSetAttribute(rollout_states_kernel<false, true, kThreads>, cudaFuncAttributeMaxDynamicSharedMemorySize, kBytes));
    NFSP_CUDA(cudaFuncSetAttribute(rollout_states_kernel<false, false, kThreads>, cudaFuncAttributeMaxDynamicSharedMemorySize, kBytes));
    return NFSP_OK;
}

int nfsp_rollout_states_configure() {
    const int rc = configure_states<kStatesThreads>();
    return rc != NFSP_OK ? rc : configure_states<kStatesThreadsSmall>();
}

int nfsp_states_ensure(nfsp_env_t h, const float *d_tab, float *d_states, cudaStream_t st) {
    if (!h->st_dirty) return NFSP_OK;
    states_pack_kernel<<<(4 * kStateQuads + 127) / 128, 128, 0, st>>>(d_tab, reinterpret_cast<float4 *>(d_states));
    NFSP_LAUNCH_CHECK();
    h->st_dirty = false;
    return NFSP_OK;
}

template <int kThreads>
static int launch_states(const RolloutArgs &A, int grid, bool debug, bool direct, cudaStream_t st) {
    constexpr int kBytes = states_smem_bytes(kThreads);
    if (debug && direct) rollout_states_kernel<true, true, kThreads><<<grid, kThreads, kBytes, st>>>(A);
    else if (debug) rollout_states_kernel<true, false, kThreads><<<grid, kThreads, kBytes, st>>>(A);
    else if (direct) rollout_states_kernel<false, true, kThreads><<<grid, kThreads, kBytes, st>>>(A);
    else rollout_states_kernel<false, false, kThreads><<<grid, kThreads, kBytes, st>>>(A);
    NFSP_LAUNCH_CHECK();
    return NFSP_OK;
}

int nfsp_rollout_states_launch(nfsp_env_t h, const RolloutArgs &A, const nfsp_rollout_io *io, bool debug, cudaStream_t st) {
    const bool direct = A.ring[0] != nullptr;
    const int sms = h->sm_count - io->reserve_sms;
    const int grid = grid_for(h->n, 32, sms, 1);
    const int64_t blocks = (h->n + 31) / 32;
    if (blocks <= (int64_t)sms * (kStatesThreadsSmall / 32)) return launch_states<kStatesThreadsSmall>(A, grid, debug, direct, st);
    return launch_states<kStatesThreads>(A, grid, debug, direct, st);
}
```

neural-ficititious-self-play-in-imperfect-information-games_b200/csrc/rollout_tables.cuh:

```cuda
#pragma once
#include "mlp_math.cuh"
#include "../../include/nfsp_b200.h"

namespace nfsp {

constexpr int kB2Floats = 4 * 4;

constexpr int kNetRows = 111, kRowQuads = 24;
constexpr int kTabRows = 4 * kNetRows;
constexpr int kTabFloats = kTabRows * kRowQuads * 4;
constexpr int kTabW2Floats = 4 * 3 * kRowQuads * 4;
constexpr int kTabImageFloats = kTabFloats + kTabW2Floats + kB2Floats;
constexpr int kTabImageBytes = kTabImageFloats * 4;

__device__ __forceinline__ uint32_t seq_bits(int rr, int d, int id) {
    const int s0 = id == 0 ? 0 : (id == 1 || id == 3 || id == 4 || id == 7 ? 1 : 2);
    const int s1 = id < 3 ? 0 : (id == 3 || id == 5 ? 1 : 2);
    const int s2 = id >= 7 ? 1 : 0;
    const int sl[3] = {s0, s1, s2};
    uint32_t bits = 0;
    for (int k = 0; k < 3; ++k)
        if (sl[k]) bits |= 1u << (((k & 1) ^ d) * 12 + rr * 6 + k * 2 + (sl[k] - 1));
    return bits;
}

__device__ __forceinline__ float pack_tables_value(const float *__restrict__ w, int e) {
    {
        float v = 0.f;
        if (e < kTabFloats) {
            const int x = e & 3, pos = (e >> 2) % kRowQuads, row = (e >> 2) / kRowQuads;
            const int net = row / kNetRows, r = row % kNetRows, j = (pos & 15) * 4 + x;
            const float *W1 = w + net * NFSP_NET_PARAMS;
            uint32_t bits = 0;
            bool bias = false;
            if (r < 3) {
                bits = 1u << (24 + r);
                bias = true;
            } else if (r < 75) {
                const int idx = r - 3, f = idx & 3, d = (idx >> 2) & 1, cp = idx >> 3, c = cp / 3, pub = cp % 3;
                const int fin[4] = {3, 5, 7, 8};
                bits = (1u << (24 + c)) | (1u << (27 + c)) | (1u << (27 + pub)) | seq_bits(0, d, fin[f]);
                bias = true;
            } else {
                bits = seq_bits(((r - 75) % 18) / 9, (r - 75) / 18, (r - 75) % 9);
            }
            for (int i = 0; i < 30; ++i)
                if ((bits >> i) & 1u) v += W1[i * 64 + j];
            if (bias) v += W1[1920 + j];
        } else if (e < kTabFloats + kTabW2Floats) {
            const int f = e - kTabFloats, x = f & 3, pos = (f >> 2) % kRowQuads, c = ((f >> 2) / kRowQuads) % 3;
            const int net = (f >> 2) / (3 * kRowQuads);
            v = w[net * NFSP_NET_PARAMS + 1984 + ((pos & 15) * 4 + x) * 3 + c];
        } else {
            const int f = e - kTabFloats - kTabW2Floats, c = f & 3, net = f >> 2;
            if (c < 3) v = w[net * NFSP_NET_PARAMS + 2176 + c];
        }
        return v;
    }
}

__device__ __forceinline__ void mlp_forward_tables(const float *__restrict__ st, uint32_t xrow, uint32_t yrow,
                                                   uint32_t net, uint32_t rot, float &o0, float &o1, float &o2) {
    const float4 *T = reinterpret_cast<const float4 *>(st);
    const float4 *xr = T + (net * kNetRows + xrow) * kRowQuads + rot;
    const float4 *yr = T + (net * kNetRows + yrow) * kRowQuads + rot;
    const float4 *wr = T + kTabRows * kRowQuads + net * (3 * kRowQuads) + rot;
    Layer2Acc acc;
#pragma unroll
    for (int q = 0; q < 16; ++q) {
        acc.quad_sum(xr[q], yr[q], wr[q], wr[kRowQuads + q], wr[2 * kRowQuads + q]);
    }
    acc.head(reinterpret_cast<const float4 *>(st + kTabFloats + kTabW2Floats)[net], net & 1u, o0, o1, o2);
}

}
```

Baseline: 50.90 billion.

## Build state table directly from weights, lazy image packing, PDL launches for rollout and insert

Setting weights now builds the variant-6 state table straight from the raw weights and only marks the packed images dirty, so they are rebuilt lazily just for the paths that use them. The states rollout kernel and the cooperative insert kernel are launched with programmatic stream serialization (griddepcontrol.wait in insert), so insert setup can overlap the tail of the rollout. Insert launch occupancy queries are cached per device. This trims the per-step weight refresh work and the launch gaps between phases, at the cost of more launch-path complexity and a fallback path when PDL plus cooperative launch is unsupported.

```diff
diff --git a/include/nfsp_b200.h b/include/nfsp_b200.h
--- a/include/nfsp_b200.h
+++ b/include/nfsp_b200.h
@@ -47,6 +47,7 @@
 int nfsp_fsm_image(uint32_t *out, int capacity_words);
 int nfsp_legacy_fsm_image(uint32_t *out, int capacity_words, int *n_rows);
 int nfsp_rollout_image(uint32_t *out, int capacity_words);
+int nfsp_rollout_states_table(nfsp_env_t h, int from_table_image, float *d_out, void *stream);
 int nfsp_env_do_action(nfsp_env_t h, const int8_t *d_actions, const int8_t *d_players, int8_t *d_fold, void *stream);
 int nfsp_env_observe(nfsp_env_t h, const int8_t *d_players, int player, uint32_t *d_s, uint32_t *d_s2,
                      float *d_reward, uint8_t *d_term, uint8_t *d_last_a, void *stream);
@@ -118,6 +119,7 @@
 int nfsp_insert_multi(const nfsp_insert_req *reqs, int n, void *stream);
 int nfsp_ring_insert_multi(const nfsp_insert_req *reqs, int n, void *stream);
 int nfsp_reservoir_insert_multi(const nfsp_insert_req *reqs, int n, void *stream);
+int nfsp_insert_launch_mode(int device);
 int nfsp_sample_indices(uint64_t seed, uint64_t call_idx, const uint64_t *d_total, int64_t cap, int is_ring,
                         int batch, int64_t *d_idx, uint32_t *d_n_out, void *stream);
 #define NFSP_MAX_SAMPLE_REQS 8
diff --git a/neural-ficititious-self-play-in-imperfect-information-games_b200/_lib.py b/neural-ficititious-self-play-in-imperfect-information-games_b200/_lib.py
--- a/neural-ficititious-self-play-in-imperfect-information-games_b200/_lib.py
+++ b/neural-ficititious-self-play-in-imperfect-information-games_b200/_lib.py
@@ -14,12 +14,12 @@
     "nfsp_version", "nfsp_last_error", "nfsp_device_info",
     "nfsp_env_create", "nfsp_env_destroy", "nfsp_env_num_games", "nfsp_env_rules", "nfsp_env_step_counter",
     "nfsp_env_set_step_counter", "nfsp_env_state_ptr", "nfsp_env_kernel_error", "nfsp_env_save_state", "nfsp_env_load_state",
-    "nfsp_env_reset", "nfsp_env_set_hands", "nfsp_env_step", "nfsp_env_do_action", "nfsp_fsm_image", "nfsp_legacy_fsm_image", "nfsp_rollout_image", "nfsp_env_observe", "nfsp_env_export",
+    "nfsp_env_reset", "nfsp_env_set_hands", "nfsp_env_step", "nfsp_env_do_action", "nfsp_fsm_image", "nfsp_legacy_fsm_image", "nfsp_rollout_image", "nfsp_rollout_states_table", "nfsp_env_observe", "nfsp_env_export",
     "nfsp_legacy_reset", "nfsp_legacy_set_hands", "nfsp_legacy_step", "nfsp_legacy_get_new_state",
     "nfsp_legacy_rollout", "nfsp_legacy_export",
     "nfsp_expand_obs",
     "nfsp_act_set_weights", "nfsp_act_set_weights_from_host", "nfsp_act_forward", "nfsp_act_forward_tc", "nfsp_rollout", "nfsp_rollout_with_weights", "nfsp_rollout_tune", "nfsp_rollout_profile",
-    "nfsp_ring_insert", "nfsp_reservoir_insert", "nfsp_insert_multi", "nfsp_ring_insert_multi", "nfsp_reservoir_insert_multi", "nfsp_sample_indices", "nfsp_sample_minibatches", "nfsp_gather_rl", "nfsp_gather_sl",
+    "nfsp_ring_insert", "nfsp_reservoir_insert", "nfsp_insert_multi", "nfsp_ring_insert_multi", "nfsp_reservoir_insert_multi", "nfsp_insert_launch_mode", "nfsp_sample_indices", "nfsp_sample_minibatches", "nfsp_gather_rl", "nfsp_gather_sl",
     "nfsp_learner_grads", "nfsp_learner_fit", "nfsp_learner_fit_peers", "nfsp_sgd_apply",
     "nfsp_peer_buffer_create", "nfsp_peer_buffer_open", "nfsp_peer_buffer_close", "nfsp_peer_buffer_destroy",
 ]
@@ -104,6 +104,7 @@
     L.nfsp_fsm_image.argtypes = [vp, C.c_int]
     L.nfsp_legacy_fsm_image.argtypes = [vp, C.c_int, vp]
     L.nfsp_rollout_image.argtypes = [vp, C.c_int]
+    L.nfsp_rollout_states_table.argtypes = [vp, C.c_int, vp, vp]
     L.nfsp_env_observe.argtypes = [vp, i8p, C.c_int, vp, vp, vp, vp, vp, vp]
     L.nfsp_env_export.argtypes = [vp, vp, vp]
     L.nfsp_legacy_reset.argtypes = [vp, vp]
@@ -124,6 +125,7 @@
     L.nfsp_insert_multi.argtypes = [C.POINTER(InsertReq), C.c_int, vp]
     L.nfsp_ring_insert_multi.argtypes = [C.POINTER(InsertReq), C.c_int, vp]
     L.nfsp_reservoir_insert_multi.argtypes = [C.POINTER(InsertReq), C.c_int, vp]
+    L.nfsp_insert_launch_mode.argtypes = [C.c_int]
     L.nfsp_sample_indices.argtypes = [C.c_uint64, C.c_uint64, vp, C.c_int64, C.c_int, C.c_int, vp, vp, vp]
     L.nfsp_sample_minibatches.argtypes = [C.POINTER(SampleReq), C.c_int, C.c_int, vp, vp, vp]
     L.nfsp_gather_rl.argtypes = [vp, vp, C.c_int, vp, vp, vp, vp, vp, vp]
diff --git a/neural-ficititious-self-play-in-imperfect-information-games_b200/csrc/act_kernels.cu b/neural-ficititious-self-play-in-imperfect-information-games_b200/csrc/act_kernels.cu
--- a/neural-ficititious-self-play-in-imperfect-information-games_b200/csrc/act_kernels.cu
+++ b/neural-ficititious-self-play-in-imperfect-information-games_b200/csrc/act_kernels.cu
@@ -34,10 +34,10 @@
 }
 
 static_assert((kPackFloats + kTabImageFloats + 4 * NFSP_NET_PARAMS) % 4 == 0, "the state table behind the images must be 16-byte aligned (bulk copy)");
+constexpr int kImageFloats = kPackFloats + kTabImageFloats;
 __global__ void pack_images_kernel(const float *__restrict__ w, float *__restrict__ pack) {
-    constexpr int kImages = kPackFloats + kTabImageFloats;
-    for (int e = blockIdx.x * blockDim.x + threadIdx.x; e < kImages + 4 * NFSP_NET_PARAMS; e += gridDim.x * blockDim.x)
-        pack[e] = e < kPackFloats ? pack_weights_value(w, e) : (e < kImages ? pack_tables_value(w, e - kPackFloats) : w[e - kImages]);
+    for (int e = blockIdx.x * blockDim.x + threadIdx.x; e < kImageFloats; e += gridDim.x * blockDim.x)
+        pack[e] = e < kPackFloats ? pack_weights_value(w, e) : pack_tables_value(w, e - kPackFloats);
 }
 
 __device__ __forceinline__ void mlp_forward(const float *__restrict__ sw, uint32_t obs, int net, uint32_t rot, float out[3]) {
@@ -181,12 +181,22 @@
         rc = nfsp_states_upload_image(h->d_states);
         if (rc != NFSP_OK) return rc;
     }
-    pack_images_kernel<<<(kPackFloats + kTabImageFloats + 4 * NFSP_NET_PARAMS + 255) / 256, 256, 0, (cudaStream_t)stream>>>(d_weights, h->d_wpack);
+    const int rc = nfsp_states_build(h, d_weights, (cudaStream_t)stream);
+    if (rc != NFSP_OK) return rc;
+    h->img_dirty = h->tc_dirty = h->tq_dirty = true;
+    h->has_weights = true;
+    return NFSP_OK;
+}
+
+int nfsp_ensure_images(nfsp_env_t h, cudaStream_t st) {
+    if (!h->img_dirty) return NFSP_OK;
+    pack_images_kernel<<<(kImageFloats + 255) / 256, 256, 0, st>>>(h->d_wcopy, h->d_wpack);
     NFSP_LAUNCH_CHECK();
-    h->tc_dirty = h->tq_dirty = h->st_dirty = true;
-    h->has_weights = true;
-    return nfsp_states_ensure(h, h->d_wpack + kPackFloats, h->d_states, (cudaStream_t)stream);
-}
+    h->img_dirty = false;
+    return NFSP_OK;
+}
+
+const float *nfsp_table_image(nfsp_env_t h) { return h->d_wpack + kPackFloats; }
 
 int nfsp_ensure_tc_images(nfsp_env_t h, bool tq, cudaStream_t st) {
     if (h->tc_dirty) {
@@ -218,6 +228,8 @@
     if (n == 0) return NFSP_OK;
     DeviceGuard guard(h->device);
     if (!guard.ok) return set_error(NFSP_E_CUDA, "cannot select device %d", h->device);
+    const int rc = nfsp_ensure_images(h, (cudaStream_t)stream);
+    if (rc != NFSP_OK) return rc;
     const int grid = grid_for(n, kActThreads, h->sm_count, 4);
     act_forward_kernel<<<grid, kActThreads, kPackFloats * sizeof(float), (cudaStream_t)stream>>>(h->d_wpack, d_obs, d_net, n, d_out);
     NFSP_LAUNCH_CHECK();
@@ -280,13 +292,15 @@
     }
     NFSP_CHECK_ARG(!direct || variant == 1 || variant >= 4, "the direct ring append (d_ring) exists in variants 1, 4, 5 and 6 only");
     if (variant == 6) {
-        int rc = nfsp_states_ensure(h, h->d_wpack + kPackFloats, h->d_states, (cudaStream_t)stream);
-        if (rc != NFSP_OK) return rc;
         A.pack = h->d_states;
-        rc = nfsp_rollout_states_launch(h, A, io, debug, (cudaStream_t)stream);
-        if (rc != NFSP_OK) return rc;
-        h->step += (uint64_t)n_steps;
-        return NFSP_OK;
+        const int rc = nfsp_rollout_states_launch(h, A, io, debug, (cudaStream_t)stream);
+        if (rc != NFSP_OK) return rc;
+        h->step += (uint64_t)n_steps;
+        return NFSP_OK;
+    }
+    if (variant == 1 || variant == 4 || variant == 5) {
+        const int rc = nfsp_ensure_images(h, (cudaStream_t)stream);
+        if (rc != NFSP_OK) return rc;
     }
     if (variant == 5) {
         const int rc = nfsp_rollout_pairs_launch(h, A, io, debug, (cudaStream_t)stream);
diff --git a/neural-ficititious-self-play-in-imperfect-information-games_b200/csrc/buffer_kernels.cu b/neural-ficititious-self-play-in-imperfect-information-games_b200/csrc/buffer_kernels.cu
--- a/neural-ficititious-self-play-in-imperfect-information-games_b200/csrc/buffer_kernels.cu
+++ b/neural-ficititious-self-play-in-imperfect-information-games_b200/csrc/buffer_kernels.cu
@@ -2,6 +2,7 @@
 
 #include "common.cuh"
 #include "philox.cuh"
+#include "ptx_helpers.cuh"
 
 namespace nfsp {
 
@@ -181,6 +182,7 @@
 constexpr int kSmallSegs = 32;
 
 __global__ void __launch_bounds__(kBufThreads, 4) insert_kernel(const MemSet S) {
+    griddep_wait();
     __shared__ uint64_t s_pre[NFSP_MAX_INSERT_REQS][kSmallSegs + 1];
     uint64_t *ctrl = S.m[0].scratch;
     uint64_t total[NFSP_MAX_INSERT_REQS], m_all[NFSP_MAX_INSERT_REQS];
@@ -440,21 +442,60 @@
     return NFSP_OK;
 }
 
+struct InsertLaunch {
+    int grid = 0;
+    int pdl = -1;
+};
+constexpr int kMaxDevices = 64;
+static InsertLaunch g_insert_launch[kMaxDevices];
+
 static int launch_insert(MemSet &S, cudaStream_t st) {
-    int dev = 0, sms = 0, per_sm = 0;
+    int dev = 0;
     NFSP_CUDA(cudaGetDevice(&dev));
-    NFSP_CUDA(cudaDeviceGetAttribute(&sms, cudaDevAttrMultiProcessorCount, dev));
-    NFSP_CUDA(cudaOccupancyMaxActiveBlocksPerMultiprocessor(&per_sm, insert_kernel, kBufThreads, 0));
-    if (per_sm < 1) return set_error(NFSP_E_CUDA, "insert_kernel does not fit an SM");
-    if (per_sm > 8) per_sm = 8;
+    NFSP_CHECK_ARG(dev >= 0 && dev < kMaxDevices, "device %d beyond the insert's launch table", dev);
+    InsertLaunch &L = g_insert_launch[dev];
+    if (L.grid == 0) {
+        int sms = 0, per_sm = 0;
+        NFSP_CUDA(cudaDeviceGetAttribute(&sms, cudaDevAttrMultiProcessorCount, dev));
+        NFSP_CUDA(cudaOccupancyMaxActiveBlocksPerMultiprocessor(&per_sm, insert_kernel, kBufThreads, 0));
+        if (per_sm < 1) return set_error(NFSP_E_CUDA, "insert_kernel does not fit an SM");
+        if (per_sm > 8) per_sm = 8;
+        L.grid = sms * per_sm;
+    }
     int64_t items = 0;
     for (int k = 0; k < S.n; ++k) items += (int64_t)S.m[k].B.n_seg * S.gx;
-    int64_t grid = (int64_t)sms * per_sm;
+    int64_t grid = L.grid;
     if (items < grid) grid = items;
     if (grid < S.n) grid = S.n;
+    if (L.pdl != 0) {
+        cudaLaunchAttribute attr[2];
+        attr[0].id = cudaLaunchAttributeCooperative;
+        attr[0].val.cooperative = 1;
+        attr[1].id = cudaLaunchAttributeProgrammaticStreamSerialization;
+        attr[1].val.programmaticStreamSerializationAllowed = 1;
+        cudaLaunchConfig_t cfg = {};
+        cfg.gridDim = dim3((unsigned)grid);
+        cfg.blockDim = dim3(kBufThreads);
+        cfg.stream = st;
+        cfg.attrs = attr;
+        cfg.numAttrs = 2;
+        const cudaError_t e = cudaLaunchKernelEx(&cfg, insert_kernel, S);
+        if (e == cudaSuccess) {
+            L.pdl = 1;
+            return NFSP_OK;
+        }
+        if (L.pdl == 1 || (e != cudaErrorInvalidValue && e != cudaErrorNotSupported))
+            return set_error(NFSP_E_CUDA, "cudaLaunchKernelEx(insert_kernel) failed: %s", cudaGetErrorString(e));
+        cudaGetLastError();
+        L.pdl = 0;
+    }
     void *args[] = {(void *)&S};
     NFSP_CUDA(cudaLaunchCooperativeKernel((const void *)insert_kernel, dim3((unsigned)grid), dim3(kBufThreads), args, 0, st));
     return NFSP_OK;
+}
+
+extern "C" int nfsp_insert_launch_mode(int device) {
+    return device >= 0 && device < kMaxDevices ? g_insert_launch[device].pdl : -1;
 }
 
 extern "C" int nfsp_insert_multi(const nfsp_insert_req *reqs, int n, void *stream) {
diff --git a/neural-ficititious-self-play-in-imperfect-information-games_b200/csrc/common.cuh b/neural-ficititious-self-play-in-imperfect-information-games_b200/csrc/common.cuh
--- a/neural-ficititious-self-play-in-imperfect-information-games_b200/csrc/common.cuh
+++ b/neural-ficititious-self-play-in-imperfect-information-games_b200/csrc/common.cuh
@@ -19,8 +19,7 @@
     uint32_t *d_work;
     void *d_wtc_wide;
     bool has_weights;
-    bool tc_dirty = false, tq_dirty = false;
-    bool st_dirty = false;
+    bool img_dirty = false, tc_dirty = false, tq_dirty = false;
     float *d_states = nullptr;
     const float *d_wcopy = nullptr;
     int w2_slot = -1;
@@ -31,6 +30,8 @@
 
 int nfsp_fsm_upload(nfsp_env_t h);
 
+int nfsp_ensure_images(nfsp_env_t h, cudaStream_t st);
+const float *nfsp_table_image(nfsp_env_t h);
 int nfsp_pack_tc_image(nfsp_env_t h, const float *d_weights, cudaStream_t st);
 int nfsp_ensure_tc_images(nfsp_env_t h, bool tq, cudaStream_t st);
 int nfsp_tq_set_weights(nfsp_env_t h, const float *d_weights, cudaStream_t st);
diff --git a/neural-ficititious-self-play-in-imperfect-information-games_b200/csrc/ptx_helpers.cuh b/neural-ficititious-self-play-in-imperfect-information-games_b200/csrc/ptx_helpers.cuh
--- a/neural-ficititious-self-play-in-imperfect-information-games_b200/csrc/ptx_helpers.cuh
+++ b/neural-ficititious-self-play-in-imperfect-information-games_b200/csrc/ptx_helpers.cuh
@@ -42,4 +42,7 @@
 }
 __device__ __forceinline__ void fence_mbar_init() { asm volatile("fence.mbarrier_init.release.cluster;" ::: "memory"); }
 
+__device__ __forceinline__ void griddep_launch_dependents() { asm volatile("griddepcontrol.launch_dependents;" ::: "memory"); }
+__device__ __forceinline__ void griddep_wait() { asm volatile("griddepcontrol.wait;" ::: "memory"); }
+
 }
diff --git a/neural-ficititious-self-play-in-imperfect-information-games_b200/csrc/rollout_common.cuh b/neural-ficititious-self-play-in-imperfect-information-games_b200/csrc/rollout_common.cuh
--- a/neural-ficititious-self-play-in-imperfect-information-games_b200/csrc/rollout_common.cuh
+++ b/neural-ficititious-self-play-in-imperfect-information-games_b200/csrc/rollout_common.cuh
@@ -14,7 +14,7 @@
 int nfsp_rollout_pairs_configure();
 
 int nfsp_rollout_states_launch(nfsp_env_t h, const nfsp::RolloutArgs &A, const nfsp_rollout_io *io, bool debug, cudaStream_t st);
-int nfsp_states_ensure(nfsp_env_t h, const float *d_tab, float *d_states, cudaStream_t st);
+int nfsp_states_build(nfsp_env_t h, const float *d_weights, cudaStream_t st);
 int nfsp_states_floats();
 int nfsp_states_upload_image(float *d_states);
 int nfsp_rollout_states_configure();
diff --git a/neural-ficititious-self-play-in-imperfect-information-games_b200/csrc/rollout_states.cu b/neural-ficititious-self-play-in-imperfect-information-games_b200/csrc/rollout_states.cu
--- a/neural-ficititious-self-play-in-imperfect-information-games_b200/csrc/rollout_states.cu
+++ b/neural-ficititious-self-play-in-imperfect-information-games_b200/csrc/rollout_states.cu
@@ -21,6 +21,26 @@
     const uint32_t sg = (uint32_t)s % 18u, x = (uint32_t)s / 18u, dl = (x >> 2) & 1u;
     xrow = sg >= 9u ? 3u + x : x / 24u;
     yrow = 75u + dl * 18u + sg;
+}
+
+__device__ __forceinline__ void state_slot(const float4 (&x)[4], const float4 (&y)[4], const float4 (&u0)[4], const float4 (&u1)[4],
+                                           const float4 (&u2)[4], const float4 &b2, uint32_t net, bool valid, int j,
+                                           float4 *__restrict__ dst) {
+    Layer2Acc acc;
+#pragma unroll
+    for (int k = 0; k < 4; ++k) acc.quad_sum(x[k], y[k], u0[k], u1[k], u2[k]);
+    float s0 = hsum2(acc.z0), s1 = hsum2(acc.z1), s2 = hsum2(acc.z2);
+#pragma unroll
+    for (int o = 1; o < 4; o <<= 1) {
+        s0 += __shfl_xor_sync(0xFFFFFFFFu, s0, o);
+        s1 += __shfl_xor_sync(0xFFFFFFFFu, s1, o);
+        s2 += __shfl_xor_sync(0xFFFFFFFFu, s2, o);
+    }
+    if (valid && j == 0) {
+        float o0, o1, o2;
+        Layer2Acc::head_of_sums(s0, s1, s2, b2, net & 1u, o0, o1, o2);
+        *dst = make_float4(o0, o1, o2, __uint_as_float(score_word(o0, o1, o2)));
+    }
 }
 
 __global__ void states_pack_kernel(const float *__restrict__ tab, float4 *__restrict__ states) {
@@ -32,24 +52,44 @@
     const float4 *T = reinterpret_cast<const float4 *>(tab);
     const float4 *xr = T + (net * kNetRows + xrow) * kRowQuads, *yr = T + (net * kNetRows + yrow) * kRowQuads;
     const float4 *wr = T + kTabRows * kRowQuads + net * (3 * kRowQuads);
-    Layer2Acc acc;
+    float4 x[4], y[4], u0[4], u1[4], u2[4];
 #pragma unroll
     for (int k = 0; k < 4; ++k) {
         const int q = j + 4 * k;
-        acc.quad_sum(xr[q], yr[q], wr[q], wr[kRowQuads + q], wr[2 * kRowQuads + q]);
-    }
-    float s0 = hsum2(acc.z0), s1 = hsum2(acc.z1), s2 = hsum2(acc.z2);
-#pragma unroll
-    for (int o = 1; o < 4; o <<= 1) {
-        s0 += __shfl_xor_sync(0xFFFFFFFFu, s0, o);
-        s1 += __shfl_xor_sync(0xFFFFFFFFu, s1, o);
-        s2 += __shfl_xor_sync(0xFFFFFFFFu, s2, o);
-    }
-    if (valid && j == 0) {
-        float o0, o1, o2;
-        Layer2Acc::head_of_sums(s0, s1, s2, reinterpret_cast<const float4 *>(tab + kTabFloats + kTabW2Floats)[net], net & 1u, o0, o1, o2);
-        states[e] = make_float4(o0, o1, o2, __uint_as_float(score_word(o0, o1, o2)));
-    }
+        x[k] = xr[q]; y[k] = yr[q]; u0[k] = wr[q]; u1[k] = wr[kRowQuads + q]; u2[k] = wr[2 * kRowQuads + q];
+    }
+    state_slot(x, y, u0, u1, u2, reinterpret_cast<const float4 *>(tab + kTabFloats + kTabW2Floats)[net], net, valid, j, states + e);
+}
+
+constexpr int kBuildThreads = 128;
+__global__ void __launch_bounds__(kBuildThreads) states_build_kernel(const float *__restrict__ w, float4 *__restrict__ states,
+                                                                     float *__restrict__ copy) {
+    const int t = blockIdx.x * blockDim.x + threadIdx.x, e = t >> 2, j = t & 3;
+    for (int k = t; k < 4 * NFSP_NET_PARAMS; k += gridDim.x * blockDim.x) copy[k] = w[k];
+    const bool valid = e < kStateQuads;
+    uint32_t xrow, yrow;
+    state_rows(valid ? e % kNetStates : 0, xrow, yrow);
+    const uint32_t net = valid ? (uint32_t)(e / kNetStates) : 0u;
+    const float *W = w + net * NFSP_NET_PARAMS;
+    int units[16];
+#pragma unroll
+    for (int u = 0; u < 16; ++u) units[u] = (j + 4 * (u >> 2)) * 4 + (u & 3);
+    float xs[16], ys[16];
+    table_row_sums(W, table_row((int)xrow), units, xs);
+    table_row_sums(W, table_row((int)yrow), units, ys);
+    float4 x[4], y[4], u0[4], u1[4], u2[4];
+#pragma unroll
+    for (int k = 0; k < 4; ++k) {
+        const int h = units[4 * k];
+        x[k] = make_float4(xs[4 * k], xs[4 * k + 1], xs[4 * k + 2], xs[4 * k + 3]);
+        y[k] = make_float4(ys[4 * k], ys[4 * k + 1], ys[4 * k + 2], ys[4 * k + 3]);
+        const float *w2 = W + 1984 + h * 3;
+        u0[k] = make_float4(w2[0], w2[3], w2[6], w2[9]);
+        u1[k] = make_float4(w2[1], w2[4], w2[7], w2[10]);
+        u2[k] = make_float4(w2[2], w2[5], w2[8], w2[11]);
+    }
+    state_slot(x, y, u0, u1, u2, make_float4(W[2176], W[2177], W[2178], 0.f), net, valid, j, states + e);
+    griddep_launch_dependents();
 }
 
 constexpr int kStatesThreads = 1024, kStatesThreadsSmall = 512;
@@ -164,6 +204,7 @@
         mbar_init(bar, 1);
         fence_mbar_init();
     }
+    griddep_wait();
     __syncthreads();
     if (threadIdx.x == 0) {
         mbar_expect_tx(bar, kStateBytes);
@@ -189,7 +230,10 @@
         uint32_t blk = 0;
         if (lane == 0) blk = blockIdx.x + gridDim.x * atomicAdd(&s_next, 1u);
         blk = __shfl_sync(0xFFFFFFFFu, blk, 0);
-        if ((int64_t)blk >= n_blocks) break;
+        if ((int64_t)blk >= n_blocks) {
+            griddep_launch_dependents();
+            break;
+        }
         const int64_t base = (int64_t)blk << 5;
         const int64_t i = base + lane;
         const bool live = i < A.n;
@@ -327,22 +371,47 @@
     return rc != NFSP_OK ? rc : configure_states<kStatesThreadsSmall>();
 }
 
-int nfsp_states_ensure(nfsp_env_t h, const float *d_tab, float *d_states, cudaStream_t st) {
-    if (!h->st_dirty) return NFSP_OK;
-    states_pack_kernel<<<(4 * kStateQuads + 127) / 128, 128, 0, st>>>(d_tab, reinterpret_cast<float4 *>(d_states));
+int nfsp_states_build(nfsp_env_t h, const float *d_weights, cudaStream_t st) {
+    states_build_kernel<<<4 * kStateQuads / kBuildThreads, kBuildThreads, 0, st>>>(d_weights, reinterpret_cast<float4 *>(h->d_states),
+                                                                               const_cast<float *>(h->d_wcopy));
     NFSP_LAUNCH_CHECK();
-    h->st_dirty = false;
+    return NFSP_OK;
+}
+static_assert(4 * kStateQuads % kBuildThreads == 0, "one lane per slot quarter, whole CTAs");
+
+extern "C" int nfsp_rollout_states_table(nfsp_env_t h, int from_table_image, float *d_out, void *stream) {
+    NFSP_CHECK_ARG(h != nullptr && d_out != nullptr, "null argument");
+    if (!h->has_weights) return set_error(NFSP_E_STATE, "nfsp_act_set_weights has not been called");
+    DeviceGuard guard(h->device);
+    if (!guard.ok) return set_error(NFSP_E_CUDA, "cannot select device %d", h->device);
+    const cudaStream_t st = (cudaStream_t)stream;
+    if (!from_table_image) {
+        NFSP_CUDA(cudaMemcpyAsync(d_out, h->d_states, (size_t)kStateBytes, cudaMemcpyDeviceToDevice, st));
+        return NFSP_OK;
+    }
+    const int rc = nfsp_ensure_images(h, st);
+    if (rc != NFSP_OK) return rc;
+    states_pack_kernel<<<4 * kStateQuads / 128, 128, 0, st>>>(nfsp_table_image(h), reinterpret_cast<float4 *>(d_out));
+    NFSP_LAUNCH_CHECK();
     return NFSP_OK;
 }
 
 template <int kThreads>
 static int launch_states(const RolloutArgs &A, int grid, bool debug, bool direct, cudaStream_t st) {
-    constexpr int kBytes = states_smem_bytes(kThreads);
-    if (debug && direct) rollout_states_kernel<true, true, kThreads><<<grid, kThreads, kBytes, st>>>(A);
-    else if (debug) rollout_states_kernel<true, false, kThreads><<<grid, kThreads, kBytes, st>>>(A);
-    else if (direct) rollout_states_kernel<false, true, kThreads><<<grid, kThreads, kBytes, st>>>(A);
-    else rollout_states_kernel<false, false, kThreads><<<grid, kThreads, kBytes, st>>>(A);
-    NFSP_LAUNCH_CHECK();
+    cudaLaunchAttribute attr[1];
+    attr[0].id = cudaLaunchAttributeProgrammaticStreamSerialization;
+    attr[0].val.programmaticStreamSerializationAllowed = 1;
+    cudaLaunchConfig_t cfg = {};
+    cfg.gridDim = dim3((unsigned)grid);
+    cfg.blockDim = dim3(kThreads);
+    cfg.dynamicSmemBytes = states_smem_bytes(kThreads);
+    cfg.stream = st;
+    cfg.attrs = attr;
+    cfg.numAttrs = 1;
+    if (debug && direct) NFSP_CUDA(cudaLaunchKernelEx(&cfg, rollout_states_kernel<true, true, kThreads>, A));
+    else if (debug) NFSP_CUDA(cudaLaunchKernelEx(&cfg, rollout_states_kernel<true, false, kThreads>, A));
+    else if (direct) NFSP_CUDA(cudaLaunchKernelEx(&cfg, rollout_states_kernel<false, true, kThreads>, A));
+    else NFSP_CUDA(cudaLaunchKernelEx(&cfg, rollout_states_kernel<false, false, kThreads>, A));
     return NFSP_OK;
 }
 
diff --git a/neural-ficititious-self-play-in-imperfect-information-games_b200/csrc/rollout_tables.cuh b/neural-ficititious-self-play-in-imperfect-information-games_b200/csrc/rollout_tables.cuh
--- a/neural-ficititious-self-play-in-imperfect-information-games_b200/csrc/rollout_tables.cuh
+++ b/neural-ficititious-self-play-in-imperfect-information-games_b200/csrc/rollout_tables.cuh
@@ -24,29 +24,44 @@
     return bits;
 }
 
+struct TableRow {
+    uint32_t bits;
+    bool bias;
+};
+__device__ __forceinline__ TableRow table_row(int r) {
+    if (r < 3) return {1u << (24 + r), true};
+    if (r < 75) {
+        const int idx = r - 3, f = idx & 3, d = (idx >> 2) & 1, cp = idx >> 3, c = cp / 3, pub = cp % 3;
+        const int fin[4] = {3, 5, 7, 8};
+        return {(1u << (24 + c)) | (1u << (27 + c)) | (1u << (27 + pub)) | seq_bits(0, d, fin[f]), true};
+    }
+    return {seq_bits(((r - 75) % 18) / 9, (r - 75) / 18, (r - 75) % 9), false};
+}
+
+template <int N>
+__device__ __forceinline__ void table_row_sums(const float *__restrict__ W1, TableRow t, const int (&units)[N], float (&v)[N]) {
+#pragma unroll
+    for (int u = 0; u < N; ++u) v[u] = 0.f;
+    for (uint32_t b = t.bits; b; b &= b - 1u) {
+        const float *row = W1 + (__ffs(b) - 1) * 64;
+#pragma unroll
+        for (int u = 0; u < N; ++u) v[u] += row[units[u]];
+    }
+    if (t.bias)
+#pragma unroll
+        for (int u = 0; u < N; ++u) v[u] += W1[1920 + units[u]];
+}
+
 __device__ __forceinline__ float pack_tables_value(const float *__restrict__ w, int e) {
     {
         float v = 0.f;
         if (e < kTabFloats) {
             const int x = e & 3, pos = (e >> 2) % kRowQuads, row = (e >> 2) / kRowQuads;
-            const int net = row / kNetRows, r = row % kNetRows, j = (pos & 15) * 4 + x;
-            const float *W1 = w + net * NFSP_NET_PARAMS;
-            uint32_t bits = 0;
-            bool bias = false;
-            if (r < 3) {
-                bits = 1u << (24 + r);
-                bias = true;
-            } else if (r < 75) {
-                const int idx = r - 3, f = idx & 3, d = (idx >> 2) & 1, cp = idx >> 3, c = cp / 3, pub = cp % 3;
-                const int fin[4] = {3, 5, 7, 8};
-                bits = (1u << (24 + c)) | (1u << (27 + c)) | (1u << (27 + pub)) | seq_bits(0, d, fin[f]);
-                bias = true;
-            } else {
-                bits = seq_bits(((r - 75) % 18) / 9, (r - 75) / 18, (r - 75) % 9);
-            }
-            for (int i = 0; i < 30; ++i)
-                if ((bits >> i) & 1u) v += W1[i * 64 + j];
-            if (bias) v += W1[1920 + j];
+            const int net = row / kNetRows, r = row % kNetRows;
+            const int j[1] = {(pos & 15) * 4 + x};
+            float s[1];
+            table_row_sums(w + net * NFSP_NET_PARAMS, table_row(r), j, s);
+            v = s[0];
         } else if (e < kTabFloats + kTabW2Floats) {
             const int f = e - kTabFloats, x = f & 3, pos = (f >> 2) % kRowQuads, c = ((f >> 2) / kRowQuads) % 3;
             const int net = (f >> 2) / (3 * kRowQuads);
diff --git a/profiles/time_step_phases.py b/profiles/time_step_phases.py
--- /dev/null
+++ b/profiles/time_step_phases.py
@@ -0,0 +1,80 @@
+import json
+import os
+import subprocess
+import sys
+
+ROOT = os.path.dirname(os.path.dirname(os.path.abspath(__file__)))
+sys.path.insert(0, ROOT)
+import torch
+
+import bench
+import nfsp_b200
+
+
+def card():
+    q = "name,power.limit,clocks.sm,clocks.max.sm"
+    try:
+        out = subprocess.run(["nvidia-smi", "-i", "0", "--query-gpu=" + q, "--format=csv,noheader"], capture_output=True,
+                             text=True, timeout=10).stdout.strip()
+    except Exception as e:
+        out = "unavailable: %r" % (e,)
+    return dict(zip(q.split(","), [f.strip() for f in out.split(",")])) if "," in out else {"nvidia-smi": out}
+
+
+def median(v):
+    v = sorted(v)
+    return v[len(v) // 2]
+
+
+def main():
+    steps = int(sys.argv[1]) if len(sys.argv) > 1 else 60
+    dev = torch.device("cuda", 0)
+    torch.cuda.set_device(dev)
+    sp = nfsp_b200.SelfPlay(bench.GAMES_PER_GPU, seed=bench.SEED, game0=0, device=dev, eta=bench.ETA, epsilon=bench.EPS,
+                            rl_capacity=bench.RL_CAP, sl_capacity=bench.SL_CAP, max_steps_per_call=bench.T_PER_CALL,
+                            variant="default", direct_rings=True)
+    flush_buf = torch.empty(256 << 20, dtype=torch.uint8, device=dev)
+    prefill = 0
+    while min(int(m.total.item()) for m in sp.sl) < bench.SL_CAP and prefill < 200:
+        sp.rollout(bench.T_PER_CALL)
+        prefill += 1
+    ev = lambda: torch.cuda.Event(enable_timing=True)
+    T = bench.T_PER_CALL
+
+    def timed(before, body):
+        before()
+        flush_buf.zero_()
+        a, b = ev(), ev()
+        a.record()
+        body()
+        b.record()
+        b.synchronize()
+        return 1e3 * a.elapsed_time(b)
+
+    nothing = lambda: None
+    staged = lambda: sp.rollout(T, insert=False)
+    rebuild, rollout, insert, whole = [], [], [], []
+    for k in range(steps + 5):
+        t = [timed(nothing, lambda: sp.set_weights(sp.weights)), timed(nothing, staged)]
+        sp.flush()
+        t.append(timed(staged, sp.flush))
+        t.append(timed(nothing, lambda: (sp.rollout(T, insert=False, refresh_weights=True), sp.flush())))
+        if k >= 5:
+            for v, x in zip((rebuild, rollout, insert, whole), t):
+                v.append(x)
+    out = {"what": "median device time per phase of a bench step (us), L2 flushed before each step",
+           "steps": steps, "games": bench.GAMES_PER_GPU, "decisions": bench.T_PER_CALL, "prefill_steps": prefill,
+           "rebuild_us": median(rebuild), "rollout_us": median(rollout), "insert_us": median(insert),
+           "whole_step_us": median(whole)}
+    out["rebuild_plus_gaps_us"] = out["whole_step_us"] - out["rollout_us"] - out["insert_us"]
+    out["reservoir_totals"] = [int(m.total.item()) for m in sp.sl]
+    try:
+        out["insert_launch_mode"] = int(nfsp_b200.lib().nfsp_insert_launch_mode(0))
+    except AttributeError:
+        out["insert_launch_mode"] = None
+    out["card"] = card()
+    print(json.dumps(out))
+
+
+if __name__ == "__main__":
+    main()
```

Measured after the change: 51.93 billion (median of 6 runs). +2.0%, better.
